# ikergarcia1996/AI-Generated-GTAV

Measured on AMD Instinct MI355X. Metric: generated frames/sec (32-frame clip, 100 noise steps), higher is better.
Workload: dtype fp16 (fp32 accumulate/residual)

## Files before the change

### ai-generated-gtav_amd/csrc/api_dit.hip

```cpp
#include "api_internal.h"

#ifdef GTAV_EXPERIMENTS
static int fold_alloc(gtav_dit* h) {
    gtav_dit::Fold& f = h->fold;
    if (f.ok) return 0;
    GTAV_REQUIRE(f.geom_ok, "dit_set_fold: this geometry has no LayerNorm fold (tokens per frame %d must be a multiple of 16 and >= 64, hidden %% 256 == 0)", h->P);
    Arena& a = h->arena;
    const int D = h->D;
    const size_t Mx = round_up(h->Mmax, 128);
    int rc = 0;
#define A_(expr) do { if (!rc) rc = (expr); } while (0)
    {
        const int nhb = h->L * 2, nseam = 2 * nhb + 1;
        f.col_c.assign(nseam, 0);
        int col = 0;
        for (int hb = 0; hb < nhb; ++hb) { f.col_c[2 * hb + 1] = col; col += 2 * h->Hm; }
        for (int hb = 0; hb < nhb; ++hb) { f.col_c[2 * hb] = col; col += 2 * 3 * D; }
        f.col_c[2 * nhb] = col; col += 2 * h->Nfin;
        f.CTW = col;
        f.n_groups = 2 * nseam; f.n_groups_a = 2 * nhb;
        f.Rp = round_up(h->max_rows, 128);
        A_(a.alloc_t(&f.ctab, (size_t)h->max_rows * f.CTW));
        A_(a.alloc_t(&f.ctab_cur, (size_t)h->maxB * h->maxT * f.CTW));
        A_(a.alloc_t(&f.stats, Mx * (size_t)(D / 64) * 2));
// ... 46 lines not shown
static int dit_fold_tables(gtav_dit* h, int rows, bool fa, bool fb, hipStream_t s) {
    if (!fa && !fb) return 0;
#ifndef GTAV_EXPERIMENTS
    (void)h; (void)rows; (void)s;
    GTAV_REQUIRE(false, "the LayerNorm fold exists only in the experiments build");
#else
    gtav_dit::Fold& f = h->fold;
    const int ng = fb ? f.n_groups : f.n_groups_a;
    RET_IF(launch_ctab_inputs(h->mod, h->MODW, rows, round_up(rows, 128), h->D, f.gcol_dev, f.gscale_dev, ng, f.sx, (size_t)f.Rp * h->D, s));
    return launch_gemm_grouped(f.groups_dev, ng, h->Hm > 3 * h->D ? h->Hm : 3 * h->D, rows, h->D, s);
#endif
}
static void fold_consumer(const gtav_dit* h, GemmParams& q, int seam, int N, const int* mod_rows, const float* ctab) {
    const gtav_dit::Fold& fo = h->fold;
    q.bias = nullptr;
    q.f_P = h->P; q.f_rows = mod_rows; q.f_stats = fo.stats; q.f_nslot = h->D / 64;
    q.f_c1 = ctab + fo.col_c[seam]; q.f_c2 = q.f_c1 + N; q.f_ldc = fo.CTW;
}
static int fold_producer(gtav_dit* h, int cls, const f16* X, const f16* Wt, int M, int K, const float* bias, const ResidGate& gt, const float* next_scale, hipStream_t s) {
    GemmParams q = gemm_params(X, K, Wt, M, h->D, K);
    q.out = h->resid; q.ldo = h->D; q.bias = bias; q.err_flag = h->err_flag;
    q.gate = gt.gate; q.gate_stride = gt.stride; q.gate_rows = gt.rows; q.rows_per_gate = gt.rows_per_gate;
    q.f_P = h->P; q.f_rows = gt.rows; q.f_scale = next_scale; q.f_stats_out = h->fold.stats; q.f_a = h->xn;
    PROF(h, cls, s, launch_gemm(q, EPI_RESID_FOLD, s));
    return 0;
}

static int dit_cond_mlp(gtav_dit* h, int rows, bool have_actions, hipStream_t s) {
    const int ldhc = h->D + h->Apad;
    RET_IF(launch_skinny_f32(h->E, 256, h->w_t0, h->b_t0, h->HC, ldhc, rows, h->D, 256, 1, s));
    RET_IF(launch_skinny_f32(h->HC, ldhc, h->w_t2cat, have_actions ? h->b_t2a : h->b_t2, h->Sc, h->D, rows, h->D, ldhc, 1, s));
    return launch_skinny_f32(h->Sc, h->D, h->w_ada, h->b_ada, h->mod, h->MODW, rows, h->MODW, h->D, 0, s);
}

static int dit_cond(gtav_dit* h, const int64_t* t64, int rows, int Tq, const StepParams* sp, int use_cur, const float* actions,
                    int64_t act_outer, int64_t act_inner, hipStream_t s) {
    GTAV_REQUIRE(rows <= h->max_rows, "conditioning rows %d exceed max_cond_rows %d", rows, h->max_rows);
    RET_IF(launch_cond_inputs(t64, rows, Tq, sp, use_cur, h->sincos, h->E, actions, act_outer, act_inner, h->A, h->HC, h->D + h->Apad,
                              h->D, h->Apad, h->err_flag, s));
    RET_IF(dit_cond_mlp(h, rows, actions != nullptr, s));
    bool fa, fb;
    fold_policy(h, rows * h->P, fa, fb);
    return dit_fold_tables(h, rows, fa, fb, s);
}

struct DitPrefetch {
    const gtav_dit* h;
    int M, Tq, t0;
    bool on;
    DitPrefetch(const gtav_dit* h_, int M_, int Tq_, int t0_) : h(h_), M(M_), Tq(Tq_), t0(t0_) {
        const int pf_max_m = 1536;
        static const int pf_min_m = GTAV_ENV_INT("GTAV_PF_MIN_M", 256);
        on = h->w_prefetch && M >= pf_min_m && M <= pf_max_m;
    }
    PrefetchDesc after(int hb, int pos) const {
        const int q = pos + 1, hb2 = hb + q / 4, consumer = (q + 3) % 4;
        if (!on || hb2 >= 2 * h->L) return kNoPrefetch;
        const int v = h->w_prefetch_cls[consumer];
        if (!v) return kNoPrefetch;
        const gtav_dit::Half& w2 = h->halves[hb2];
        const int D = h->D;
        const f16* W; int N, K, sk = 1;
        if (consumer == 3) { W = dit_half_fused(h, hb2, M, Tq, t0) ? w2.w_qkv_hm : w2.w_qkv; N = 3 * D; K = D; }
        else if (consumer == 0) { W = w2.w_out; N = D; K = D; sk = gemm_choose_splitk(M, D, D); }
        else if (consumer == 1) { W = w2.w_fc1; N = h->Hm; K = D; }
        else { W = w2.w_fc2; N = D; K = h->Hm_pad; sk = gemm_choose_splitk(M, D, h->Hm_pad); }
        const int nkt = K / 64;
        if (sk < 1 || nkt % sk || (sk >= 8 ? sk % 8 : 8 % sk)) sk = 1;
        return PrefetchDesc{W, cdiv(N, 128), nkt, sk, v >= 2 ? v : 0};
    }
};

static bool dit_resid_inplace(const gtav_dit* h, int M, int K) {
    return gemm_pp_ok(M, h->D, K, EPI_RESID) || (gemm_choose_splitk(M, h->D, K) == 1 && M >= h->resid_inplace_min_m) || gemm_resid_inplace_ok(M, h->D, K, h->P);
}

static int dit_forward_core(gtav_dit* h, const float* x_src, const int* frame_index, int B, int Tq, int t0,
                            const float* mod, const int* mod_rows, const float* ctab, float* v_out, hipStream_t s) {
    const int D = h->D, P = h->P, NB = B * Tq, M = NB * P;
    GTAV_REQUIRE(M <= h->Mmax, "forward: %d tokens exceed workspace (%d)", M, h->Mmax);
    bool fold_a, fold_b;
    fold_policy(h, M, fold_a, fold_b);
    const DitPrefetch pf(h, M, Tq, t0);
    DeferredResid rd{h->parts, h->parts_rows * (size_t)D, h->resid, M, D, &h->prof, s};
    auto gate = [&](const float* g) { return ResidGate{g, h->MODW, mod_rows, P}; };
    auto ln = [&](const OperandOps& o, const float* shift, const float* scale, int* ef) -> int {
        PROF(h, PC_LN, s, o.ln_modulate(h->resid, D, h->xn, D, M, D, shift, scale, h->MODW, mod_rows, P, rd.take(), ef, s));
        return 0;
    };
    const int g_embed = 2 * h->L, g_final = 2 * h->L + 1;
    PROF(h, PC_OTHER, s, h->ops(g_embed).patchify(x_src, frame_index, NB, h->C, h->H, h->W, h->p, h->xp, h->Kpe, 1.f, 0.f, h->err_of(g_embed), s));
    GemmParams pe = gemm_params(h->xp, h->Kpe, h->w_pe, M, D, h->Kpe);
    pe.bias = h->b_pe; pe.out = h->resid; pe.ldo = D;
    PROF(h, PC_OTHER, s, h->ops(g_embed).gemm(pe, EPI_F32, s));
    bool folded_in = false;
    for (int hb = 0; hb < 2 * h->L; ++hb) {
        const int l = hb / 2, hf = hb % 2;
        const gtav_dit::Half& w = h->halves[hb];
        const OperandOps& ops = h->ops(hb);
        int* const ef = h->err_of(hb);
        const float* mb = mod + (size_t)hb * 6 * D;
        const bool fused = dit_half_fused(h, hb, M, Tq, t0), fused_t = fused && hf == 1, fused_s = fused && hf == 0 && !folded_in;
        if (fused_t) rd.permute_rows(Tq, P);
        if (!folded_in) RET_IF(ln(ops, mb, mb + D, ef));
        GemmParams g = gemm_params(h->xn, D, fused_t || fused_s ? w.w_qkv_hm : w.w_qkv, M, 3 * D, D);
        g.D = D; g.S = P; g.err_flag = ef; g.pf = pf.after(hb, 0);
        if (folded_in) fold_consumer(h, g, 2 * hb, 3 * D, mod_rows, ctab);
        if (hf == 0) { g.qkv_mode = QKV_SPATIAL; g.rope_cs = h->rope_s.cs_dev; }
        else { g.qkv_mode = QKV_TEMPORAL; g.k = h->kvcache[l]; g.v = h->kvcache[l]; g.Tq = Tq; g.t0 = t0; g.Tmax = h->maxT; g.rope_cs = h->rope_t.cs_dev; }
        if (fused_t || fused_s) {
            g.out = h->ao; g.ldo = D;
            if (fused_t) PROF(h, PC_ATTN_T, s, launch_gemm_qkvt_attn(g, s));
            else PROF(h, PC_ATTN_S, s, launch_gemm_qkvs_attn(g, s));
        } else {
            if (hf == 0) { g.q = h->qs; g.k = h->ks; g.v = h->vts; }
            else g.q = h->qt;
            PROF(h, PC_QKV, s, ops.gemm(g, folded_in ? EPI_QKV_FOLD : EPI_QKV, s));
            if (hf == 0) PROF(h, PC_ATTN_S, s, ops.attn_spatial(h->qs, h->ks, h->vts, h->ao, NB, h->heads, P, s, false));
            else PROF(h, PC_ATTN_T, s, ops.attn_temporal(h->qt, h->kvcache[l], h->ao, B, P, D, Tq, t0, h->maxT, s));
        }
        folded_in = false;
        GemmParams fc1 = gemm_params(h->xn, D, w.w_fc1, M, h->Hm, D);
        fc1.bias = w.b_fc1; fc1.out = h->hbuf; fc1.ldo = h->Hm_pad; fc1.err_flag = ef; fc1.pf = pf.after(hb, 2);
        if (fold_a) {
            RET_IF(fold_producer(h, PC_OUT, h->ao, w.w_out, M, D, w.b_out, gate(mb + 2 * D), mb + 4 * D, s));
            fold_consumer(h, fc1, 2 * hb + 1, h->Hm, mod_rows, ctab);
            PROF(h, PC_FC1, s, launch_gemm(fc1, EPI_GELU_TANH_FOLD, s));
        } else {
            RET_IF(rd.gemm(ops, PC_OUT, h->ao, D, w.w_out, D, w.b_out, gate(mb + 2 * D), dit_resid_inplace(h, M, D), pf.after(hb, 1)));
            RET_IF(ln(ops, mb + 3 * D, mb + 4 * D, ef));
            PROF(h, PC_FC1, s, ops.gemm(fc1, EPI_GELU_TANH, s));
        }
        if (fold_b) {
            const float* next_scale = hb + 1 < 2 * h->L ? mod + (size_t)(hb + 1) * 6 * D + D : mod + (size_t)h->L * 12 * D + D;
            RET_IF(fold_producer(h, PC_FC2, h->hbuf, w.w_fc2, M, h->Hm_pad, w.b_fc2, gate(mb + 5 * D), next_scale, s));
            folded_in = true;
        } else {
            RET_IF(rd.gemm(ops, PC_FC2, h->hbuf, h->Hm_pad, w.w_fc2, h->Hm_pad, w.b_fc2, gate(mb + 5 * D), dit_resid_inplace(h, M, h->Hm_pad), pf.after(hb, 3)));
        }
    }
    const float* mf = mod + (size_t)h->L * 12 * D;
    if (!folded_in) RET_IF(ln(h->ops(g_final), mf, mf + D, h->err_of(g_final)));
    GemmParams fin = gemm_params(h->xn, D, h->w_final, M, h->Nfin, D);
    fin.bias = h->b_final; fin.out = h->fo; fin.ldo = h->Nfin;
    if (folded_in) fold_consumer(h, fin, 4 * h->L, h->Nfin, mod_rows, ctab);
    PROF(h, PC_OTHER, s, h->ops(g_final).gemm(fin, folded_in ? EPI_F32_FOLD : EPI_F32, s));
    PROF(h, PC_OTHER, s, launch_unpatchify(h->fo, h->Nfin, v_out, NB, h->C, h->H, h->W, h->p, 0, 1.f, 0.f, s));
    return h->prof.collect(s);
}

extern "C" {

int gtav_dit_create(const gtav_dit_config* c, gtav_dit** out) {
    GTAV_REQUIRE(c && out, "dit_create: null argument");
    GTAV_REQUIRE(c->hidden_size % 256 == 0 && c->hidden_size <= 2048, "hidden_size=%d must be a multiple of 256, <= 2048", c->hidden_size);
    GTAV_REQUIRE(c->num_heads > 0 && c->hidden_size / c->num_heads == 64 && c->hidden_size % c->num_heads == 0,
                 "only head_dim 64 is implemented (hidden %d, heads %d)", c->hidden_size, c->num_heads);
    GTAV_REQUIRE(c->input_h % c->patch_size == 0 && c->input_w % c->patch_size == 0, "input %dx%d not divisible by patch %d",
                 c->input_h, c->input_w, c->patch_size);
    GTAV_REQUIRE(c->max_frames >= 1 && c->max_frames <= 32, "max_frames=%d must be in [1, 32]", c->max_frames);
    GTAV_REQUIRE(c->max_batch >= 1 && c->depth >= 1, "bad max_batch/depth");
    RET_IF(skinny_init());
    gtav_dit* h = new gtav_dit();
    h->cfg = *c;
    h->D = c->hidden_size; h->L = c->depth; h->heads = c->num_heads; h->C = c->in_channels; h->p = c->patch_size;
    h->H = c->input_h; h->W = c->input_w; h->gh = h->H / h->p; h->gw = h->W / h->p; h->P = h->gh * h->gw;
    const int D = h->D;
    if ((h->P % 8) != 0) {
        set_error("tokens per frame P=%d must be a multiple of 8", h->P);
        delete h;
        return 2;
    }
    h->Hm = (int)(D * c->mlp_ratio); h->Hm_pad = round_up(h->Hm, 128);
    h->A = c->external_cond_dim > 0 ? c->external_cond_dim : 0; h->Apad = round_up(h->A > 0 ? h->A : 1, 32);
    h->MODW = h->L * 12 * D + 2 * D;
    h->Kpe = round_up(h->C * h->p * h->p, 64);
    h->Nfin = h->p * h->p * h->C;
    h->maxB = c->max_batch; h->maxT = c->max_frames; h->Mmax = h->maxB * h->maxT * h->P;
    h->max_rows = c->max_cond_rows > h->maxB * h->maxT ? c->max_cond_rows : h->maxB * h->maxT;
    Arena& a = h->arena;
    WeightTable& wt = h->wt;
    int rc = 0;
#define A_(expr) do { if (!rc) rc = (expr); } while (0)
    A_(a.alloc_t(&h->w_pe, (size_t)round_up(D, 128) * h->Kpe));
    h->n_groups = 2 * h->L + 2;
    h->grp_bf16.assign(h->n_groups, 0);
    wt.add_f16("x_embedder.proj.weight", D, h->C * h->p * h->p, h->w_pe, round_up(D, 128), h->Kpe, 2 * h->L);
    A_(a.alloc_t(&h->b_pe, D)); wt.add_f32("x_embedder.proj.bias", 1, D, h->b_pe, D);
    A_(a.alloc_t(&h->w_t0, (size_t)D * 256)); wt.add_f32("t_embedder.mlp.0.weight", D, 256, h->w_t0, 256);
    A_(a.alloc_t(&h->b_t0, D)); wt.add_f32("t_embedder.mlp.0.bias", 1, D, h->b_t0, D);
    const int ldhc = D + h->Apad;
// ... 237 lines not shown
    GTAV_REQUIRE(t_cur >= 0 && t_cur < 1000 && t_next >= 0 && t_next < 1000 && t_ctx >= 0 && t_ctx < 1000, "denoise_step: timestep out of range");
    GTAV_REQUIRE(!actions || h->A > 0, "denoise_step: model has no external_cond");
    GTAV_REQUIRE(mode == 0 || mode == 1, "denoise_step: mode %d", mode);
    const bool prepared = cond_step >= 0;
    if (prepared)
        GTAV_REQUIRE(h->prepared.valid && h->prepared.B == B && h->prepared.F == F && h->prepared.start == start &&
                         h->prepared.cur == cur && cond_step < h->prepared.n_steps && h->prepared.actions == actions,
                     "denoise_step: cond_step=%d but gtav_dit_prepare_frame was not called for this window", cond_step);
    else
        h->prepared.valid = false;
    if (mode == 1) {
        GTAV_REQUIRE(h->kvrec.valid && h->kvrec.B == B && h->kvrec.F == F && h->kvrec.start == start && h->kvrec.cur == cur &&
                         h->kvrec.x == (const void*)x,
                     "denoise_step: context-cached step (mode 1) on window [%d, %d] without a preceding full-window step (mode 0) "
                     "on the same batch / window / latent buffer: the temporal K/V caches would be stale", start, cur);
    } else {
        h->kvrec.valid = true; h->kvrec.B = B; h->kvrec.F = F; h->kvrec.start = start; h->kvrec.cur = cur; h->kvrec.x = x;
    }
    hipStream_t s = (hipStream_t)stream;
    StepParams sp;
    sp.first = start; sp.cur = cur; sp.t_ctx = t_ctx; sp.t_cur = t_cur; sp.is_final = is_final != 0;
    sp.alpha_t = h->ac_host[t_cur]; sp.alpha_next = h->ac_host[t_next]; sp.cond_step = cond_step;
    RET_IF(launch_step_setup(h->step_dev, sp, h->frame_idx, h->mod_rows_dev, prepared ? h->mod_last : nullptr, h->mod_changed, B, mode == 1 ? 1 : T, T, F,
                             mode == 1, s));
    if (prepared) RET_IF(launch_gather_rows(h->mod, h->mod_rows_dev, h->mod_changed, h->mod_cur, B * (mode == 1 ? 1 : T), h->MODW,
                                            h->prepared.fold_tables ? h->fold.ctab : nullptr, h->fold.ctab_cur, h->fold.CTW, s));
    hipGraphExec_t exec = nullptr;
    if (h->use_graph && !h->prof.on) RET_IF(dit_step_graph(h, x, B, F, T, actions, mode, v_out, prepared, &exec));
    if (!exec) return denoise_step_body(h, x, B, F, T, actions, mode, v_out, prepared, s);
    GTAV_CHECK_HIP(hipGraphLaunch(exec, s));
    return 0;
}

int gtav_dit_set_graph(gtav_dit* h, int32_t enable) {
    GTAV_REQUIRE(h, "dit_set_graph: null handle");
    h->use_graph = enable != 0;
    return 0;
}

int gtav_dit_set_weight_prefetch(gtav_dit* h, int32_t enable) {
    GTAV_REQUIRE(h, "dit_set_weight_prefetch: null handle");
    GTAV_REQUIRE(enable == 0 || enable == 1 || (enable >> 16) == 1,
                 "dit_set_weight_prefetch: mode %d (0 off, 1 on, 0x10000 | per-class nibbles: bits 0-3 out-proj's weight, 4-7 fc1's, 8-11 fc2's, 12-15 to_qkv's; "
                 "nibble 0 = not prefetched, 1 = the whole slice, k >= 2 = the first k K tiles of every row tile)", enable);
    int cls[4];
    for (int c = 0; c < 4; ++c) cls[c] = enable == 0 ? 0 : enable == 1 ? 1 : (enable >> (4 * c)) & 15;
    const bool on = cls[0] || cls[1] || cls[2] || cls[3];
    if (h->w_prefetch != on || memcmp(cls, h->w_prefetch_cls, sizeof(cls))) h->drop_graphs();
    h->w_prefetch = on;
    memcpy(h->w_prefetch_cls, cls, sizeof(cls));
    return 0;
}

#ifdef GTAV_EXPERIMENTS
int gtav_dit_set_fold(gtav_dit* h, int32_t mode, int32_t min_tokens_a, int32_t min_tokens_b) {
    GTAV_REQUIRE(h && mode >= 0 && mode <= 2, "dit_set_fold: mode %d", mode);
    if (min_tokens_a >= 0) h->fold.min_m_a = min_tokens_a;
    if (min_tokens_b >= 0) h->fold.min_m_b = min_tokens_b;
    if (mode == 2 || (mode == 1 && (h->fold.min_m_a < (1 << 30) || h->fold.min_m_b < (1 << 30)))) RET_IF(fold_alloc(h));
    h->drop_graphs();
    h->prepared.valid = false;
    h->fold.mode = mode;
    return 0;
}
#endif

static int dit_set_fused(gtav_dit* h, bool& flag, int hf, bool geom_ok, bool enable) {
    if (flag != enable) h->drop_graphs();
    if (enable && geom_ok) {
        for (int l = 0; l < h->L; ++l) {
            gtav_dit::Half& w = h->halves[l * 2 + hf];
            if (w.w_qkv_hm) continue;
            RET_IF(h->arena.alloc_t(&w.w_qkv_hm, (size_t)3 * h->D * h->D));
            if (h->finalized) RET_IF(launch_qkv_head_major(w.w_qkv, w.w_qkv_hm, h->D, nullptr, hf ? 0 : 1));
        }
        if (h->finalized) GTAV_CHECK_HIP(hipDeviceSynchronize());
    }
    flag = enable;
    return 0;
}
int gtav_dit_set_fused_temporal(gtav_dit* h, int32_t enable) {
    GTAV_REQUIRE(h, "dit_set_fused_temporal: null handle");
    return dit_set_fused(h, h->fuse_tattn, 1, h->P % 16 == 0 && h->D % 256 == 0 && h->maxT >= 5, enable != 0);
}
int gtav_dit_set_fused_spatial(gtav_dit* h, int32_t enable) {
    GTAV_REQUIRE(h, "dit_set_fused_spatial: null handle");
    return dit_set_fused(h, h->fuse_sattn, 0, h->P == 144 && h->D % 256 == 0, enable != 0);
}

int gtav_dit_fused_launches(gtav_dit* h, int32_t B, int32_t T, int32_t t0) {
    if (!h || B < 1 || T < 1) return 0;
    int mask = 0;
    for (int hb = 0; hb < 2 * h->L; ++hb)
        if (dit_half_fused(h, hb, B * T * h->P, T, t0)) mask |= (hb & 1) ? 2 : 1;
    return mask;
}

int gtav_dit_profile(gtav_dit* h, int32_t enable) {
    GTAV_REQUIRE(h, "dit_profile: null handle");
    h->prof.reset(enable != 0);
    return 0;
}
int gtav_dit_profile_read(gtav_dit* h, double* ms_by_class, int64_t* launches_by_class) {
    GTAV_REQUIRE(h && ms_by_class && launches_by_class, "dit_profile_read: null argument");
    h->prof.read(ms_by_class, launches_by_class);
    return 0;
// ... 74 lines not shown
```

### ai-generated-gtav_amd/csrc/api_internal.h

```cpp
#pragma once
#include "../../include/gtav_amd.h"
#include "../../include/gtav_amd_testing.h"
#include "ops.h"
#include "ops_bf16.h"

#include <cmath>
#include <cstdarg>
#include <cstdio>
#include <cstdlib>
#include <cstring>
#include <map>
#include <string>
#include <tuple>
#include <vector>

using namespace gtav;

#define RET_IF(expr)            \
    do {                        \
        int _rc = (expr);       \
        if (_rc) return _rc;    \
    } while (0)

namespace gtav {
// ... 181 lines not shown
            GTAV_CHECK_HIP(hipEventElapsedTime(&t, ev[i], ev[i + 1]));
            ms[cls[i / 2]] += t;
            n[cls[i / 2]] += 1;
        }
        used = 0;
        return 0;
    }
    void reset(bool enable) {
        on = enable;
        used = 0;
        for (int i = 0; i < PC_COUNT; ++i) { ms[i] = 0; n[i] = 0; }
    }
    void read(double* ms_by_class, int64_t* launches_by_class) const {
        for (int i = 0; i < PC_COUNT; ++i) { ms_by_class[i] = ms[i]; launches_by_class[i] = n[i]; }
    }
    ~Profiler() {
        for (hipEvent_t e : ev) (void)hipEventDestroy(e);
    }
};
#define PROF(h, c, s, expr)            \
    do {                               \
        RET_IF((h)->prof.begin(c, s)); \
        RET_IF(expr);                  \
        RET_IF((h)->prof.end(s));      \
    } while (0)

inline int report_err_flag(int flag, const char* who) {
    GTAV_REQUIRE(!(flag & ERR_TIMESTEP), "%s: a timestep outside [0, 999] was passed", who);
    GTAV_REQUIRE(!(flag & ERR_NONFINITE), "%s: a NaN or inf was found in the input tensor", who);
    GTAV_REQUIRE(!(flag & ERR_F16_SAT), "%s: an activation exceeded the fp16 range (|x| > 65504) and was saturated; results since the "
                 "last check are finite but clipped (the reference runs this path in bf16, which has fp32 range)", who);
    return 0;
}

inline GemmParams gemm_params(const f16* X, int ldx, const f16* W, int M, int N, int K) {
    GemmParams g;
    memset(&g, 0, sizeof(g));
    g.X = X; g.ldx = ldx; g.W = W; g.M = M; g.N = N; g.K = K;
    return g;
}

const PrefetchDesc kNoPrefetch{nullptr, 0, 0, 0, 0};

struct ResidGate { const float* gate; int stride; const int* rows; int rows_per_gate; };
struct DeferredResid {
    float* parts; size_t parts_floats;
    float* resid;
    int M, N;
    Profiler* prof;
    hipStream_t s;
    LnPending pend;
    bool pending = false;
    int gemm(const OperandOps& ops, int cls, const f16* X, int ldx, const f16* W, int K, const float* bias, const ResidGate& gt, bool inplace,
             const PrefetchDesc& pf = kNoPrefetch, float* x_out = nullptr, f16* y_save = nullptr) {
        GemmParams q = gemm_params(X, ldx, W, M, N, K);
        q.out = parts; q.ldo = N; q.pf = pf;
        if (inplace) {
            q.out = resid; q.bias = bias; q.gate = gt.gate; q.gate_stride = gt.stride; q.gate_rows = gt.rows; q.rows_per_gate = gt.rows_per_gate;
        } else {
            q.splitk = gemm_choose_splitk(M, N, K);
            GTAV_REQUIRE((size_t)q.splitk * M * N <= parts_floats, "split-K slabs exceed workspace");
        }
        if (prof) RET_IF(prof->begin(cls, s));
        RET_IF(ops.gemm(q, inplace ? EPI_RESID : EPI_PARTIAL, s));
        if (prof) RET_IF(prof->end(s));
        pending = !inplace;
        if (inplace) return 0;
        memset(&pend, 0, sizeof(pend));
        pend.parts = parts; pend.nsplit = q.splitk; pend.slab_stride = (size_t)M * N; pend.ld = N; pend.bias = bias;
        pend.gate = gt.gate; pend.gate_stride = gt.stride; pend.gate_rows = gt.rows; pend.rows_per_gate = gt.rows_per_gate;
        pend.x_out = x_out; pend.y_save = y_save;
        return 0;
    }
    const LnPending* take() {
        const bool was = pending;
        pending = false;
        return was ? &pend : nullptr;
    }
    void permute_rows(int T, int P) {
        if (!pending) memset(&pend, 0, sizeof(pend));
        pend.tperm_T = T; pend.tperm_P = P;
        pending = true;
    }
    void save_shift(float* k) { pend.k_save = k; }
    int load_shift(const float* k) {
        GTAV_REQUIRE(!pending, "train_block_forward: a re-run starts from a stored block input");
        memset(&pend, 0, sizeof(pend));
        pend.k_load = k;
        pending = true;
        return 0;
    }
};

}
}
using namespace gtav::api;

struct gtav_dit {
    Profiler prof;
    gtav_dit_config cfg;
    int D, L, heads, P, gh, gw, C, p, H, W, Hm, Hm_pad, A, Apad, MODW, Kpe, Nfin, maxB, maxT, Mmax, max_rows;
    Arena arena;
    WeightTable wt;
    f16 *w_pe = nullptr, *w_final = nullptr;
    struct Half { f16 *w_qkv, *w_out, *w_fc1, *w_fc2; float *b_out, *b_fc1, *b_fc2; f16* w_qkv_hm; };
    std::vector<Half> halves;
    float *b_pe = nullptr, *b_final = nullptr;
    float *w_t0, *b_t0, *w_t2cat, *b_t2, *b_ext, *b_t2a, *w_ada, *b_ada;
    float* sincos = nullptr;
    bool sincos_set = false;
    RopeTable rope_s, rope_t;
    std::vector<float> freqs_s, freqs_t;
    float *freqs_s_dev = nullptr, *freqs_t_dev = nullptr;
    f16 *xp, *xn, *qs, *ks, *vts, *qt, *ao, *hbuf;
    std::vector<f16*> kvcache;
    float *resid, *fo, *vout, *E, *HC, *Sc, *mod, *parts;
    size_t parts_rows = 0;
    int* err_flag = nullptr;
    std::vector<unsigned char> grp_bf16;
    int n_groups = 0;
    bool any_bf16 = false;
    const OperandOps& ops(int g) const { return operand_ops(grp_bf16[g] != 0); }
    int* err_of(int g) const { return err_flag + 4 + g; }
    int* frame_idx = nullptr;
    StepParams* step_dev = nullptr;
    int* mod_rows_dev = nullptr;
    float* mod_cur = nullptr;
    int *mod_last = nullptr, *mod_changed = nullptr;
    int* t_steps_dev = nullptr;
    struct { bool valid = false, fold_tables = false; int B = 0, F = 0, start = 0, cur = 0, n_steps = 0; const float* actions = nullptr; } prepared;
    struct { bool valid = false; int B = 0, F = 0, start = 0, cur = 0; const void* x = nullptr; } kvrec;
    struct GraphKey {
        int B, F, T, mode;
        const void *x, *actions, *vout;
        bool operator<(const GraphKey& o) const {
            return std::tie(B, F, T, mode, x, actions, vout) < std::tie(o.B, o.F, o.T, o.mode, o.x, o.actions, o.vout);
        }
    };
    std::map<GraphKey, hipGraphExec_t> graphs;
    bool use_graph = true;
    bool fuse_tattn = false;
    bool fuse_sattn = false;
    bool w_prefetch = true;
    int w_prefetch_cls[4] = {1, 4, 4, 1};
    int resid_inplace_min_m = GTAV_ENV_INT("GTAV_RESID_INPLACE_MIN_M", 1 << 30);
    struct Fold {
        bool geom_ok = false;
        bool ok = false;
        int mode = 1;
        int min_m_a = 1 << 30, min_m_b = 1 << 30;
        int CTW = 0, n_groups = 0, n_groups_a = 0, Rp = 0;
        std::vector<int> col_c;
        float *ctab = nullptr, *ctab_cur = nullptr, *stats = nullptr;
        f16* sx = nullptr;
        GemmGroup* groups_dev = nullptr;
        int *gcol_dev = nullptr, *gscale_dev = nullptr;
    } fold;
    hipStream_t cap_stream = nullptr;
    void drop_graphs() {
        for (auto& kv : graphs)
            if (kv.second) (void)hipGraphExecDestroy(kv.second);
        graphs.clear();
    }
    ~gtav_dit() {
        drop_graphs();
        if (cap_stream) (void)hipStreamDestroy(cap_stream);
    }
    float* ac_table = nullptr;
    std::vector<float> ac_host;
    bool finalized = false;
    struct Train {
        bool on = false, have_fwd = false, have_actions = false;
        bool bf16 = false;
        int window = 8;
        bool recompute = false;
        int rc_block = -1;
        std::vector<float*> kshift;
        size_t saved_bytes = 0;
        int B = 0, T = 0, M = 0, Mp = 0, rows = 0;
        float loss_scale = 65536.0f;
        float grad_div = 1.0f;
        std::vector<Slot*> params;
        struct Linear { Slot *w = nullptr, *b = nullptr; };
        struct HalfSlots { Linear qkv, out, fc1, fc2, ada; };
        std::vector<HalfSlots> hs;
        Linear fin, fin_ada, pe, t0, t2, ext;
        float* grad_arena = nullptr;
        size_t grad_count = 0;
        float* ctl = nullptr;
        float *ln_part = nullptr;
        float *red_ws = nullptr, *sumsq_part = nullptr;
        size_t red_ws_floats = 0;
        AdamParam* adam_params = nullptr;
        AdamItem* adam_items = nullptr;
        int adam_n_items = 0;
        std::vector<float*> res;
        struct HB { f16 *xnA, *ao, *y1, *xnB, *u, *hh, *y2, *q, *k, *v; };
// ... 10 lines not shown
```

### ai-generated-gtav_amd/csrc/elementwise.hip

```cpp
#include "ops.h"

#include <cstdlib>
#include <type_traits>

#include <cstring>

namespace gtav {

namespace {

template <int MODE, int NV>
__global__ __launch_bounds__(256) void ln_wave_row_kernel(const float* __restrict__ x, int ldx, f16* __restrict__ out, int M, int D,
                                                          const float* __restrict__ p0, const float* __restrict__ p1, int mod_stride,
                                                          const int* __restrict__ rows, int rows_per_mod, int flags, int* err_flag) {
    const int lane = threadIdx.x & 63;
    const int m = blockIdx.x * 4 + (threadIdx.x >> 6);
    if (m >= M) return;
    const float* xr = x + (size_t)m * ldx;
    f32x4 v[NV], av[NV], bv[NV];
#pragma unroll
    for (int i = 0; i < NV; ++i) v[i] = *(const f32x4*)(xr + i * 256 + lane * 4);
    const float *a, *b;
    if (MODE == 0) {
        int row = m / rows_per_mod;
        if (rows) row = rows[row];
        a = p1 + (size_t)row * mod_stride;
        b = p0 + (size_t)row * mod_stride;
    } else {
        a = p0;
        b = p1;
    }
#pragma unroll
    for (int i = 0; i < NV; ++i) {
        av[i] = *(const f32x4*)(a + i * 256 + lane * 4);
        bv[i] = *(const f32x4*)(b + i * 256 + lane * 4);
    }
    const float kshift = __builtin_bit_cast(float, __builtin_amdgcn_readfirstlane(__builtin_bit_cast(int, v[0][0])));
    float s1 = 0.f, s2 = 0.f;
#pragma unroll
    for (int i = 0; i < NV; ++i) {
        const float a0 = v[i][0] - kshift, a1 = v[i][1] - kshift, a2 = v[i][2] - kshift, a3 = v[i][3] - kshift;
        s1 += (a0 + a1) + (a2 + a3);
        s2 += (a0 * a0 + a1 * a1) + (a2 * a2 + a3 * a3);
    }
    const float t1 = wave_sum_dpp(s1), t2 = wave_sum_dpp(s2);
    const float m1 = t1 / (float)D;
    const float var = fmaxf(t2 / (float)D - m1 * m1, 0.f);
    const float rstd = 1.0f / sqrtf(var + 1e-6f);
    float amax = 0.f;
#pragma unroll
    for (int i = 0; i < NV; ++i) {
        float yv[4];
#pragma unroll
        for (int e = 0; e < 4; ++e) {
            const float xh = ((v[i][e] - kshift) - m1) * rstd;
            if (MODE == 0) {
                const float sc = av[i][e] + 1e-6f;
                yv[e] = xh * (1.0f + sc) + bv[i][e];
            } else {
                yv[e] = xh * av[i][e] + bv[i][e];
            }
        }
        store_f16x4_paired<1>(out + tiled_off(m, i * 256 + lane * 4, D), sat4(yv[0], yv[1], yv[2], yv[3], amax), lane, flags & 2);
    }
    sat_report(amax, err_flag);
}

#ifdef GTAV_EXPERIMENTS
#define LN_DBG(pd, b) ((pd).flags & (b))
#else
#define LN_DBG(pd, b) false
#endif
template <int MODE, bool PEND, int KS = 0>
__global__ __launch_bounds__(512) void ln_row_block_kernel(float* __restrict__ x, int ldx, f16* __restrict__ out, int M, int D,
                                                           const float* __restrict__ p0, const float* __restrict__ p1,
                                                           int mod_stride, const int* __restrict__ rows, int rows_per_mod,
                                                           LnPending pd) {
    __shared__ float red[16];
    const int m = blockIdx.x;
    const int c = threadIdx.x * 4;
    const int nw = (blockDim.x + 63) >> 6, wid = threadIdx.x >> 6, lane = threadIdx.x & 63;
    float* xr = x + (size_t)m * ldx;
    const bool act = c < D;
    const bool nt = PEND && (pd.flags & 4);
    f32x4 v = f32x4{0.f, 0.f, 0.f, 0.f}, av = v, bv = v;
    if (act) v = nt ? __builtin_nontemporal_load((const f32x4*)(xr + c)) : *(const f32x4*)(xr + c);
    f32x4 sl[8];
    int nchunk = 0;
    if (PEND && act) {
        const float* pp = pd.parts + (size_t)m * pd.ld + c;
        auto slab = [&](int sp) -> f32x4 {
            const f32x4* q = (const f32x4*)(pp + (size_t)sp * pd.slab_stride);
            return nt ? __builtin_nontemporal_load(q) : *q;
        };
        nchunk = pd.nsplit <= 1 ? 1 : pd.nsplit <= 2 ? 2 : pd.nsplit <= 4 ? 4 : 8;
        if (nchunk == 1) {
            sl[0] = slab(0);
        } else if (nchunk == 2) {
#pragma unroll
            for (int sp = 0; sp < 2; ++sp) sl[sp] = slab(sp < pd.nsplit ? sp : 0);
        } else if (nchunk == 4) {
#pragma unroll
            for (int sp = 0; sp < 4; ++sp) sl[sp] = slab(sp < pd.nsplit ? sp : 0);
        } else {
#pragma unroll
            for (int sp = 0; sp < 8; ++sp) sl[sp] = slab(sp < pd.nsplit ? sp : 0);
        }
    }
    int row = 0, gr = 0;
    if (MODE == 0) {
        row = m / rows_per_mod;
        if (rows && !LN_DBG(pd, 0x2000)) row = rows[row];
    }
    if (PEND && pd.gate) {
        gr = m / pd.rows_per_gate;
        if (pd.gate_rows && !LN_DBG(pd, 0x2000)) gr = pd.gate_rows[gr];
    }
    const float kshift = LN_DBG(pd, 0x200) ? 0.f : KS == 2 ? pd.k_load[m] : xr[0];
    if (act && !LN_DBG(pd, 0x100)) {
        av = *(const f32x4*)((MODE == 0 ? p1 + (size_t)row * mod_stride : p0) + c);
        bv = *(const f32x4*)((MODE == 0 ? p0 + (size_t)row * mod_stride : p1) + c);
    }
    if (PEND && act) {
        f32x4 y = pd.bias && !LN_DBG(pd, 0x100) ? *(const f32x4*)(pd.bias + c) : f32x4{0.f, 0.f, 0.f, 0.f};
        f32x4 g4 = f32x4{1.f, 1.f, 1.f, 1.f};
        if (pd.gate && !LN_DBG(pd, 0x100)) g4 = *(const f32x4*)(pd.gate + (size_t)gr * pd.gate_stride + c);
#pragma unroll
        for (int sp = 0; sp < 8; ++sp)
            if (sp < nchunk && sp < pd.nsplit) y = y + sl[sp];
        if (pd.y_save) {
            float am = 0.f;
// ... 520 lines not shown
                else v = ((const float*)src)[(((size_t)f * 3 + c) * H + (y0 + a)) * W + (x0 + j)];
                row += aa_w(x0 + j, cx, ix) * v;
            }
            acc += wy * row;
        }
        dst[idx] = acc / (wxs * wys) * in_scale;
    }
}

inline int grid_for(size_t total, int block = 256) {
    size_t g = (total + block - 1) / block;
    if (g > 256 * 16) g = 256 * 16;
    if (g < 1) g = 1;
    return (int)g;
}

__global__ void qkv_head_major_kernel(const f16* __restrict__ src, f16* __restrict__ dst, int D, int mode) {
    const size_t i = (size_t)blockIdx.x * blockDim.x + threadIdx.x;
    const int cpr = D >> 3;
    if (i >= (size_t)3 * D * cpr) return;
    const int nd = (int)(i / cpr), kc = (int)(i - (size_t)nd * cpr);
    const int hd = nd / 192, rem = nd - hd * 192;
    int which, d;
    if (mode == 0) {
        which = rem >> 6;
        d = rem & 63;
    } else {
        const int w = rem / 48, r48 = rem - w * 48;
        which = r48 >> 4;
        d = 16 * w + (r48 & 15);
    }
    const int ns = which * D + hd * 64 + d;
    *(uint4*)(dst + tiled_off(nd, kc * 8, D)) = *(const uint4*)(src + tiled_off(ns, kc * 8, D));
}

__global__ void calib_spin_kernel(unsigned long long ticks, unsigned long long* __restrict__ dev_ticks) {
    const unsigned long long t0 = __builtin_amdgcn_s_memrealtime();
    unsigned long long t1 = t0;
    while (t1 - t0 < ticks) {
        __builtin_amdgcn_s_sleep(2);
        t1 = __builtin_amdgcn_s_memrealtime();
    }
    if (threadIdx.x == 0) dev_ticks[0] = t1 - t0;
}

}

static int g_ln_flags = GTAV_ENV_INT("GTAV_LN_FLAGS", 7);

static int g_ln_wave_row_min = GTAV_ENV_INT("GTAV_LN_WAVE_ROW_MIN", 0);

#define LN_WAVE_ROW_(MODE, NV, P0, P1, STRIDE, ROWS, RPM) \
    GTAV_LAUNCH((ln_wave_row_kernel<MODE, NV>), dim3(cdiv(M, 4)), dim3(256), 0, stream, x, ldx, out, M, D, P0, P1, STRIDE, ROWS, RPM, pd_.flags, err_flag)
#define LN_DISPATCH(MODE, P0, P1, STRIDE, ROWS, RPM)                                                     \
    do {                                                                                                  \
        LnPending pd_;                                                                                    \
        memset(&pd_, 0, sizeof(pd_));                                                                     \
        if (pend) pd_ = *pend;                                                                            \
        pd_.flags = g_ln_flags;                                                                           \
        pd_.err_flag = err_flag;                                                                          \
        GTAV_REQUIRE(pd_.tperm_T == 0 || (pd_.tperm_P % 16 == 0 && M % (pd_.tperm_T * pd_.tperm_P) == 0), "ln: bad output row permutation"); \
        const bool upd_ = pend && pend->parts;    \
        GTAV_REQUIRE(!pd_.k_save || (upd_ && !pd_.k_load), "ln: k_save needs a pending update and excludes k_load");                          \
        GTAV_REQUIRE(!pd_.k_load || !upd_, "ln: k_load excludes a pending update");                                                            \
        if (pd_.k_save || pd_.k_load) {                  \
            const dim3 g_(M), b_(round_up(D / 4, 64));                                                    \
            if (pd_.k_save) GTAV_LAUNCH((ln_row_block_kernel<MODE, true, 1>), g_, b_, 0, stream, x, ldx, out, M, D, P0, P1, STRIDE, ROWS, RPM, pd_); \
            else GTAV_LAUNCH((ln_row_block_kernel<MODE, false, 2>), g_, b_, 0, stream, x, ldx, out, M, D, P0, P1, STRIDE, ROWS, RPM, pd_);      \
        } else if (!upd_ && pd_.tperm_T == 0 && M >= g_ln_wave_row_min && (D == 256 || D == 512 || D == 1024 || D == 2048)) { \
            if (D == 256) LN_WAVE_ROW_(MODE, 1, P0, P1, STRIDE, ROWS, RPM);                               \
            else if (D == 512) LN_WAVE_ROW_(MODE, 2, P0, P1, STRIDE, ROWS, RPM);                          \
            else if (D == 1024) LN_WAVE_ROW_(MODE, 4, P0, P1, STRIDE, ROWS, RPM);                         \
            else LN_WAVE_ROW_(MODE, 8, P0, P1, STRIDE, ROWS, RPM);                                        \
        } else {                                                                   \
            const dim3 g_(M), b_(round_up(D / 4, 64));                                                    \
            if (upd_) GTAV_LAUNCH((ln_row_block_kernel<MODE, true>), g_, b_, 0, stream, x, ldx, out, M, D, P0, P1, STRIDE, ROWS, RPM, pd_); \
            else GTAV_LAUNCH((ln_row_block_kernel<MODE, false>), g_, b_, 0, stream, x, ldx, out, M, D, P0, P1, STRIDE, ROWS, RPM, pd_);     \
        }                                                                                                 \
    } while (0)

int launch_ln_modulate(float* x, int ldx, f16* out, int ldo, int M, int D, const float* shift, const float* scale,
                       int mod_stride, const int* rows, int rows_per_mod, const LnPending* pend, int* err_flag, hipStream_t stream) {
    GTAV_REQUIRE(D % 64 == 0 && D <= 2048 && rows_per_mod > 0 && ldo == D, "ln_modulate: D=%d must be %%64, <= 2048, ldo == D", D);
    GTAV_REQUIRE(!pend || !pend->parts || (pend->nsplit >= 1 && pend->nsplit <= 8 && pend->ld % 4 == 0 && (!pend->gate || pend->rows_per_gate > 0)),
                 "ln_modulate: bad pending update");
    LN_DISPATCH(0, shift, scale, mod_stride, rows, rows_per_mod);
    GTAV_CHECK_HIP(hipGetLastError());
    return 0;
}

int launch_ln_affine(float* x, int ldx, f16* out, int ldo, int M, int D, const float* gamma, const float* beta,
                     const LnPending* pend, int* err_flag, hipStream_t stream) {
    GTAV_REQUIRE(D % 64 == 0 && D <= 2048 && ldo == D, "ln_affine: D=%d must be %%64, <= 2048, ldo == D", D);
    GTAV_REQUIRE(!pend || !pend->parts || (pend->nsplit >= 1 && pend->nsplit <= 8 && pend->ld % 4 == 0 && (!pend->gate || pend->rows_per_gate > 0)),
                 "ln_affine: bad pending update");
    LN_DISPATCH(1, gamma, beta, 0, (const int*)nullptr, 1);
    GTAV_CHECK_HIP(hipGetLastError());
    return 0;
}
#undef LN_DISPATCH
#undef LN_WAVE_ROW_

int launch_patchify(const float* img, const int* frame_index, int NB, int C, int H, int W, int p, f16* out, int ldo,
                    float a, float b, int* err_flag, hipStream_t stream) {
    GTAV_REQUIRE(H % p == 0 && W % p == 0 && ldo >= C * p * p, "patchify: bad geometry");
    const size_t total = (size_t)NB * (H / p) * (W / p) * ldo;
    if (p % 4 == 0 && W % 4 == 0 && ldo % 4 == 0 && ((uintptr_t)img & 15) == 0 && (size_t)NB * (H / p) * (W / p) < (1u << 31)) {
        hipLaunchKernelGGL(patchify4_kernel, dim3(NB * (H / p) * (W / p)), dim3(256), 0, stream, img, frame_index, C, H, W, p, out, ldo, a, b, err_flag);
        GTAV_CHECK_HIP(hipGetLastError());
        return 0;
    }
    hipLaunchKernelGGL(patchify_kernel, dim3(grid_for(total)), dim3(256), 0, stream, img, frame_index, NB, C, H, W, p, out,
                       ldo, a, b, err_flag);
    GTAV_CHECK_HIP(hipGetLastError());
    return 0;
}

int launch_unpatchify(const float* y, int ldy, float* img, int NB, int C, int H, int W, int p, int order, float a,
                      float b, hipStream_t stream) {
    GTAV_REQUIRE(H % p == 0 && W % p == 0 && ldy >= C * p * p, "unpatchify: bad geometry");
    const size_t total = (size_t)NB * C * H * W;
    hipLaunchKernelGGL(unpatchify_kernel, dim3(grid_for(total)), dim3(256), 0, stream, y, ldy, img, NB, C, H, W, p, order,
                       a, b);
    GTAV_CHECK_HIP(hipGetLastError());
    return 0;
}

int launch_convert_pad_f16(const float* src, int lds, int R, int C, f16* dst, int Rp, int Cp, float scale, int tiled,
                           hipStream_t stream, int* err_flag) {
    GTAV_REQUIRE(Rp >= R && Cp >= C, "convert_pad: padded shape smaller than source");
// ... 206 lines not shown
```

### ai-generated-gtav_amd/csrc/gemm.hip

```cpp
#include "gemm.h"
#include "attn_tile.h"

#include <cstdlib>
#include <cstring>
#include <type_traits>
#include <hip/hip_ext.h>

namespace gtav {

namespace {

constexpr int TN = 128, TK = 64;
constexpr int TILE_BYTES = 128 * TK * 2;

typedef const __attribute__((address_space(1))) void* gptr_t;
typedef __attribute__((address_space(3))) void* lptr_t;

__device__ __forceinline__ void glds16(const char* src, char* lds_wave_base) {
    __builtin_amdgcn_global_load_lds((gptr_t)src, (lptr_t)lds_wave_base, 16, 0, 0);
}

__device__ __forceinline__ void glds16_s(const void* sbase, unsigned voff, unsigned lds_addr) {
    unsigned keep;
    asm volatile("s_mov_b32 %0, m0\n\ts_mov_b32 m0, %3\n\ts_nop 0\n\tglobal_load_lds_dwordx4 %1, %2\n\ts_mov_b32 m0, %0"
                 : "=&s"(keep) : "v"(voff), "s"(sbase), "s"(lds_addr) : "memory");
}
__device__ __forceinline__ void store16_soff(const void* sbase, unsigned voff, u32x4 v) {
    asm volatile("global_store_dwordx4 %0, %1, %2" : : "v"(voff), "v"(v), "s"(sbase) : "memory");
}
__device__ __forceinline__ void glds4_s(const void* sbase, unsigned voff, unsigned lds_addr) {
    unsigned keep;
    asm volatile("s_mov_b32 %0, m0\n\ts_mov_b32 m0, %3\n\ts_nop 0\n\tglobal_load_lds_dword %1, %2\n\ts_mov_b32 m0, %0"
                 : "=&s"(keep) : "v"(voff), "s"(sbase), "s"(lds_addr) : "memory");
}
__device__ __forceinline__ unsigned lds_offset(const void* p) { return (unsigned)(size_t)(lptr_t)p; }

__device__ __forceinline__ void store16q_sc1(void* dst, uint4 v) { store16_sc1(dst, u32x4{v.x, v.y, v.z, v.w}); }

__device__ __forceinline__ uint2 pack4(float& amax, float a, float b, float c, float d) {
    union { f16x4 h; uint2 u; } cv;
    cv.h = sat4(a, b, c, d, amax);
    return cv.u;
}


constexpr int waitcnt_imm(int vm, int lgkm) { return (vm & 15) | (7 << 4) | ((lgkm & 15) << 8) | ((vm >> 4) << 14); }
__device__ __forceinline__ f32x4 rope4(const f32x4 v, const f32x4 cs) {
    f32x4 r;
    r[0] = __builtin_fmaf(v[0], cs[0], -(v[1] * cs[1]));
    r[1] = __builtin_fmaf(v[1], cs[0], v[0] * cs[1]);
    r[2] = __builtin_fmaf(v[2], cs[2], -(v[3] * cs[3]));
    r[3] = __builtin_fmaf(v[3], cs[2], v[2] * cs[3]);
    return r;
}

__device__ __forceinline__ const float* rope_tab(const GemmParams& p, int n) { return (p.rope_cs_q && n < p.D) ? p.rope_cs_q : p.rope_cs; }

template <int VM>
__device__ __forceinline__ void wait_vm() {
    static_assert(VM >= 0 && VM < 64, "vmcnt is a 6-bit field");
    __builtin_amdgcn_s_waitcnt(waitcnt_imm(VM, 15));
}
__device__ __forceinline__ void wait_lgkm0() { __builtin_amdgcn_s_waitcnt(waitcnt_imm(63, 0)); }
__device__ __forceinline__ void wg_barrier() { asm volatile("s_barrier" ::: "memory"); }
template <int VM>
__device__ __forceinline__ void kstep_sync() {
    wait_lgkm0();
    wait_vm<VM>();
    wg_barrier();
}
template <int NS, int G>
__device__ __forceinline__ void wait_vm_ring(int rem) {
    if constexpr (NS >= 6) { if (rem >= 4) { wait_vm<4 * G>(); return; } }
    if constexpr (NS >= 5) { if (rem >= 3) { wait_vm<3 * G>(); return; } }
    if constexpr (NS >= 4) { if (rem >= 2) { wait_vm<2 * G>(); return; } }
    if constexpr (NS >= 3) { if (rem >= 1) { wait_vm<G>(); return; } }
    wait_vm<0>();
// ... 412 lines not shown
            __builtin_amdgcn_sched_barrier(0);
        }
        {
            sync(nkt - 1);
            f16x8 wf[2][FI], xf[2][FJ];
            rd(nkt - 1, wf, xf);
            per_step(nkt - 1);
            mm(wf, xf);
        }
    } else {
        for (int t = 0; t < nkt; ++t) {
            sync(t);
            const bool refill = t + NS - 1 < nkt && !GTAV_DBG(p, 1);
            if (refill && !late) stage(t + NS - 1);
            per_step(t);
            f16x8 wf[2][FI], xf[2][FJ];
            rd(t, wf, xf);
            mm(wf, xf);
            if (refill && late) {
                asm volatile("" ::: "memory");
                stage(t + NS - 1);
            }
        }
    }
}

template <bool SPLITK, int TNB, int TMB>
__device__ __forceinline__ void tile_map(const GemmParams& p, int& n0, int& m0, int& ks, int& kt0, int& nkt) {
    const int tiles_m = (p.M + TMB - 1) / TMB, tiles_n = (p.N + TNB - 1) / TNB;
    const int nwg = gridDim.x, bid = blockIdx.x;
    const int xcd = bid & 7, qq = nwg >> 3, rr = nwg & 7;
    const int swz = (xcd < rr ? xcd * (qq + 1) : rr * (qq + 1) + (xcd - rr) * qq) + (bid >> 3);
    int tile_id = swz;
    ks = 0, kt0 = 0, nkt = p.K / TK;
    if constexpr (SPLITK) {
        const int tiles = tiles_m * tiles_n;
        ks = swz / tiles;
        tile_id = swz - ks * tiles;
        nkt = nkt / p.splitk;
        kt0 = ks * nkt;
    }
    int gn = p.tm.gn;
    const int group = tiles_m * gn;
    const int ng = tile_id / group, rem = tile_id - ng * group;
    const int n_first = ng * gn;
    if (n_first + gn > tiles_n) gn = tiles_n - n_first;
    const int tile_m = rem / gn, tile_n = n_first + (rem - tile_m * gn);
    n0 = tile_n * TNB;
    m0 = tile_m * TMB;
}

__device__ __forceinline__ int div_rcp(int a, unsigned rcp) { return rcp ? (int)__umulhi((unsigned)a, rcp) : a; }
template <bool SPLITK, int TNB, int TMB>
__device__ __forceinline__ void tile_map_fast(const GemmParams& p, int& n0, int& m0, int& ks, int& kt0, int& nkt) {
    const GemmParams::TileMap& tm = p.tm;
    const int nwg = gridDim.x, bid = blockIdx.x;
    const int xcd = bid & 7, qq = nwg >> 3, rr = nwg & 7;
    const int swz = (xcd < rr ? xcd * (qq + 1) : rr * (qq + 1) + (xcd - rr) * qq) + (bid >> 3);
    int tile_id = swz;
    ks = 0, kt0 = 0, nkt = p.K / TK;
    if constexpr (SPLITK) {
        ks = div_rcp(swz, tm.rcp_tiles);
        tile_id = swz - ks * tm.tiles;
        nkt = nkt / p.splitk;
        kt0 = ks * nkt;
    }
    const int ng = div_rcp(tile_id, tm.rcp_group), rem = tile_id - ng * tm.group;
    const int n_first = ng * tm.gn;
    const bool last = n_first + tm.gn > tm.tiles_n;
    const int gn = last ? tm.tiles_n - n_first : tm.gn;
    const int tile_m = div_rcp(rem, last ? tm.rcp_gnlast : tm.rcp_gn), tile_n = n_first + (rem - tile_m * gn);
    n0 = tile_n * TNB;
    m0 = tile_m * TMB;
}

constexpr int FOLD_NFR = 4;
constexpr int fold_lds_bytes(int tnb) { return FOLD_NFR * 2 * tnb * 4; }
template <int FJ>
struct FoldTok {
    float mu[FJ], rs[FJ];
    int b1, b2, b3;
    int kmax;
    int nchunk;
    f32x4 tpre;
    const char* cb;
};
template <int FJ>
__device__ __forceinline__ int fold_frame_of(const FoldTok<FJ>& ft, int m) {
    const int k = (m >= ft.b1 ? 1 : 0) + (m >= ft.b2 ? 1 : 0) + (m >= ft.b3 ? 1 : 0);
    return k < ft.kmax ? k : ft.kmax;
}
template <int TNB, int TM, int FJ>
__device__ __forceinline__ void fold_prefetch(const GemmParams& p, int n0, int m0, int ct , int mw ,
                                              bool compute_wave, FoldTok<FJ>& ft) {
    const int mlast = m0 + TM - 1 < p.M ? m0 + TM - 1 : p.M - 1;
    const int f_first = m0 / p.f_P, nfr = mlast / p.f_P - f_first + 1;
    ft.b1 = (f_first + 1) * p.f_P; ft.b2 = ft.b1 + p.f_P; ft.b3 = ft.b2 + p.f_P;
    ft.kmax = nfr - 1;
    constexpr int Q = TNB / 4;
    ft.nchunk = nfr * 2 * Q;
    ft.tpre = f32x4{0.f, 0.f, 0.f, 0.f};
    ft.cb = nullptr;
    if (ct >= 0 && ct < ft.nchunk) {
        const int k = ct / (2 * Q), r = ct - k * 2 * Q, t = r / Q, n4 = r - t * Q;
        int n = n0 + 4 * n4;
        n = n < p.N ? n : p.N - 4;
        const int row = p.f_rows ? p.f_rows[f_first + k] : f_first + k;
        ft.tpre = *(const f32x4*)((t ? p.f_c2 : p.f_c1) + (size_t)row * p.f_ldc + n);
    }
    if (!compute_wave) return;
    const int lane = threadIdx.x & 63, li = lane & 15, g = lane >> 4;
    const int q = p.f_nslot >> 2;
    const float inv_d = 1.0f / (float)(p.f_nslot * 64);
#pragma unroll
    for (int j = 0; j < FJ; ++j) {
        int m = mw + 16 * j + li;
        m = m < p.M ? m : p.M - 1;
        const float* sp = p.f_stats + ((size_t)m * p.f_nslot + g * q) * 2;
        float a1 = 0.f, a2 = 0.f;
        if (q & 1) {
            for (int s = 0; s < q; ++s) {
                const float2 v = *(const float2*)(sp + 2 * s);
                a1 += v.x; a2 += v.y;
            }
        } else {
            for (int s = 0; s < q; s += 2) {
                const f32x4 v = *(const f32x4*)(sp + 2 * s);
// ... 936 lines not shown
    else if constexpr (FOLDC || FOLDP) epilogue<EPIX, FI, FJ, WM, 2, 0, false>(p, acc, pbias, smem, n0, m0, ks, tr, acc, ft);
    else epilogue<EPIX, FI, FJ, WM>(p, acc, pbias, smem, n0, m0, ks, tr);
    bs.end(p);
}

template <int NS, int FI, int FJ, int WM>
__global__ __launch_bounds__(128 * WM, 1) void gemm_grouped_kernel(GemmParams p0, const GemmGroup* __restrict__ groups) {
    constexpr int TNB = 32 * FI, TM = 16 * FJ * WM;
    constexpr int STAGE = (4 * FI + 2 * FJ * WM) * 1024;
    __shared__ __attribute__((aligned(16))) char smem[NS * STAGE];
    GemmParams p = p0;
    {
        const GemmGroup* gr = groups + blockIdx.y;
        p.X = gr->X; p.W = gr->W; p.out = gr->out; p.bias = gr->bias; p.N = gr->N; p.ldo = gr->ldo;
    }
    const int tiles_m = (p.M + TM - 1) / TM, tiles_n = (p.N + TNB - 1) / TNB, tiles = tiles_m * tiles_n;
    const int bid = blockIdx.x;
    if (bid >= tiles) return;
    const int xcd = bid & 7, qq = tiles >> 3, rr = tiles & 7;
    const bool inrange = (bid >> 3) < qq + (xcd < rr ? 1 : 0);
    const int tile_id = inrange ? (xcd < rr ? xcd * (qq + 1) : rr * (qq + 1) + (xcd - rr) * qq) + (bid >> 3) : bid;
    const int tile_m = tile_id / tiles_n, tile_n = tile_id - tile_m * tiles_n;
    const int n0 = tile_n * TNB, m0 = tile_m * TM;
    BlockStamps bs;
    f32x4 acc[FI][FJ];
#pragma unroll
    for (int i = 0; i < FI; ++i)
#pragma unroll
        for (int j = 0; j < FJ; ++j) acc[i][j] = f32x4{0.f, 0.f, 0.f, 0.f};
    f32x4 pbias[FI];
    auto pf = [&]() { prefetch_bias<EPI_F32, FI, WM>(p, n0, pbias); };
    mainloop_g<false, NS, FI, FJ, WM>(p, smem, n0, m0, 0, p.K / TK, acc, bs, pf);
    epilogue<EPI_F32, FI, FJ, WM>(p, acc, pbias, smem, n0, m0, 0, false);
}

template <bool TR, int NS, int FI, int FJ, int WN, int WM, int NL, int TRI = FI, bool HALFSTEP = (FI * FJ >= 16), typename AfterPrologue>
__device__ __forceinline__ void mainloop_l(const GemmParams& p, char* smem, int n0, int m0, int kt0, int nkt,
                                           f32x4 (&acc)[FI][FJ], BlockStamps& bs, AfterPrologue after_prologue) {
    static_assert(NS >= 3 && NL >= 1, "loader-wave ring: at least 3 stages and one loader wave");
    constexpr int NCW = WN * WM;
    constexpr int WPC = 2 * FI * WN, XPC = 2 * FJ * WM, NP = WPC + XPC;
    constexpr int G = (NP + NL - 1) / NL;
    constexpr int STAGE_BYTES = NP * 1024;
    const int tid = threadIdx.x, lane = tid & 63;
    const int wraw = __builtin_amdgcn_readfirstlane(tid >> 6);
    const int nktot = p.K / TK;
    if (wraw < NL) {
        const int lw = wraw;
        const int last_wt = ((p.N + 127) >> 7) - 1, last_rt = (p.M - 1) >> 7;
        const unsigned voff = (unsigned)lane * 16u;
        const unsigned smem0 = lds_offset(smem);
        const char* sb[G];
        unsigned ldso[G];
#pragma unroll
        for (int i = 0; i < G; ++i) {
            int q = lw * G + i;
            q = q < NP ? q : NP - 1;
            const bool isw = q < WPC;
            const int row = isw ? n0 + 8 * q : m0 + 8 * (q - WPC);
            int rt = row >> 7;
            const int lim = isw ? last_wt : last_rt;
            rt = rt < lim ? rt : lim;
            sb[i] = (const char*)(isw ? p.W : p.X) + ((size_t)rt * nktot + kt0) * TILE_BYTES + ((row & 127) >> 3) * 1024;
            ldso[i] = smem0 + q * 1024;
        }
        auto stage = [&](int t) {
            const unsigned so = (unsigned)(t % NS) * STAGE_BYTES;
            const size_t go = (size_t)t * TILE_BYTES;
#pragma unroll
            for (int i = 0; i < G; ++i) glds16_s(sb[i] + go, voff, ldso[i] + so);
        };
        const int npro = nkt < NS - 1 ? nkt : NS - 1;
        GTAV_STAMP_SLOT(lw == 0 && lane == 0, 7);
        for (int t = 0; t < npro; ++t) stage(t);
        for (int t = 0; t < nkt; ++t) {
            wait_vm_ring<NS, G>(nkt - 1 - t);
            GTAV_STAMP_SLOT_HI(t == 0 && lw == 0 && lane == 0, 6);
            wg_barrier();
            if (t == 0) GTAV_STAMP(bs.t[1]);
            GTAV_STAMP_SLOT(GTAV_DBG(p, 32) && lw == 0 && lane == 0 && t < 24, 8 + t);
            if (t + NS - 1 < nkt && !GTAV_DBG(p, 1)) stage(t + NS - 1);
        }
        return;
    }
    const int w = wraw - NL;
    const int wn = w % WN, wm = w / WN;
    const int li = lane & 15, g = lane >> 4;
    int woff[2], xoff[2];
#pragma unroll
    for (int s = 0; s < 2; ++s) {
        const int ch = ((4 * s + g) ^ (li & 7)) << 4;
        woff[s] = (16 * FI * wn + li) * 128 + ch;
        xoff[s] = WPC * 1024 + (16 * FJ * wm + li) * 128 + ch;
    }
    l2_prefetch_next(p, w, NCW, lane, bs.pf_sink);
    after_prologue();
    auto rd = [&](int t, f16x8 (&wf)[2][FI], f16x8 (&xf)[2][FJ]) {
        const char* b = smem + (t % NS) * STAGE_BYTES;
#pragma unroll
        for (int s = 0; s < 2; ++s) {
#pragma unroll
            for (int i = 0; i < FI; ++i) wf[s][i] = *(const f16x8*)(b + woff[s] + i * 16 * 128);
#pragma unroll
            for (int j = 0; j < FJ; ++j) xf[s][j] = *(const f16x8*)(b + xoff[s] + j * 16 * 128);
        }
    };
    auto mm = [&](const f16x8 (&wf)[2][FI], const f16x8 (&xf)[2][FJ]) {
#pragma unroll
        for (int s = 0; s < 2; ++s)
#pragma unroll
            for (int i = 0; i < FI; ++i)
#pragma unroll
                for (int j = 0; j < FJ; ++j) {
                    if (TR || i >= TRI) acc[i][j] = mfma16(xf[s][j], wf[s][i], acc[i][j], 0, 0, 0);
                    else acc[i][j] = mfma16(wf[s][i], xf[s][j], acc[i][j], 0, 0, 0);
                }
    };
    if constexpr (HALFSTEP) {
        f16x8 wa[FI], xa[FJ], wb[FI], xb[FJ];
        auto rdh = [&](int t, int sh, f16x8 (&wf)[FI], f16x8 (&xf)[FJ]) {
            const char* b = smem + (t % NS) * STAGE_BYTES;
#pragma unroll
            for (int i = 0; i < FI; ++i) wf[i] = *(const f16x8*)(b + woff[sh] + i * 16 * 128);
#pragma unroll
            for (int j = 0; j < FJ; ++j) xf[j] = *(const f16x8*)(b + xoff[sh] + j * 16 * 128);
        };
// ... 6 lines not shown
                    else acc[i][j] = mfma16(wf[i], xf[j], acc[i][j], 0, 0, 0);
                }
        };
        const bool domm = !GTAV_DBG(p, 2);
        for (int t = 0; t < nkt; ++t) {
            wait_lgkm0();
            wg_barrier();
            if (t == 0) GTAV_STAMP(bs.t[1]);
            if (t > 0) {
                rdh(t, 0, wa, xa);
                if (domm) mmh(wb, xb);
                interleave_mfma_dsread<FI * FJ, FI + FJ>();
            } else {
                rdh(t, 0, wa, xa);
            }
            __builtin_amdgcn_sched_barrier(0);
            rdh(t, 1, wb, xb);
            if (domm) mmh(wa, xa);
            interleave_mfma_dsread<FI * FJ, FI + FJ>();
            __builtin_amdgcn_sched_barrier(0);
        }
        if (domm) mmh(wb, xb);
    } else {
        f16x8 wA[2][FI], xA[2][FJ], wB[2][FI], xB[2][FJ];
        auto step = [&](int t, f16x8 (&wr)[2][FI], f16x8 (&xr)[2][FJ], const f16x8 (&wm_)[2][FI], const f16x8 (&xm_)[2][FJ]) {
            GTAV_STAMP_SLOT(GTAV_DBG(p, 32) && w == 0 && lane == 0 && t < 24, 32 + t);
            wait_lgkm0();
            wg_barrier();
            if (t == 0) GTAV_STAMP(bs.t[1]);
            if (t > 0 && !GTAV_DBG(p, 2)) {
                rd(t, wr, xr);
                mm(wm_, xm_);
                interleave_mfma_dsread<2 * FI * FJ, 2 * (FI + FJ), 1>();
            } else {
                rd(t, wr, xr);
            }
            __builtin_amdgcn_sched_barrier(0);
        };
        int t = 0;
        for (; t + 1 < nkt; t += 2) {
            step(t, wA, xA, wB, xB);
            step(t + 1, wB, xB, wA, xA);
        }
        if (t < nkt) {
            step(t, wA, xA, wB, xB);
            if (!GTAV_DBG(p, 2)) mm(wA, xA);
        } else if (!GTAV_DBG(p, 2)) {
            mm(wB, xB);
        }
    }
}

template <int EPIX, int NS, int FI, int FJ, int WN, int WM, int NL>
__global__ __launch_bounds__(64 * (WN * WM + NL), 1) void gemm_l_kernel(GemmParams p) {
    constexpr int EPI = epi_base(EPIX);
    constexpr int TNB = 16 * FI * WN, TM = 16 * FJ * WM;
    constexpr int STAGE = (2 * FI * WN + 2 * FJ * WM) * 1024;
    constexpr int PNB = (TNB / 8 + 7) / 8 * 8 * 16, PTB = (TM / 8 + 7) / 8 * 8 * 16;
    constexpr int EPIB = (TM * PNB > TNB * PTB ? TM * PNB : TNB * PTB) + TM * 8 + (epi_is_fold_consumer(EPIX) ? fold_lds_bytes(TNB) : 0);
    extern __shared__ __attribute__((aligned(16))) char smem_l[];
    static_assert(NS * STAGE >= EPIB, "the ring must cover the epilogue's LDS image");
    char* smem = smem_l;
#define GTAV_PIN_S(x) asm volatile("" ::"s"(x))
    GTAV_PIN_S(p.X); GTAV_PIN_S(p.W); GTAV_PIN_S(p.M); GTAV_PIN_S(p.N); GTAV_PIN_S(p.K); GTAV_PIN_S(p.splitk);
    GTAV_PIN_S(p.tm.tiles_m); GTAV_PIN_S(p.tm.tiles_n); GTAV_PIN_S(p.tm.gn); GTAV_PIN_S(p.tm.group); GTAV_PIN_S(p.tm.tiles);
    GTAV_PIN_S(p.tm.rcp_tiles); GTAV_PIN_S(p.tm.rcp_group); GTAV_PIN_S(p.tm.rcp_gn); GTAV_PIN_S(p.tm.rcp_gnlast);
    GTAV_PIN_S(p.bias); GTAV_PIN_S(p.out); GTAV_PIN_S(p.ldo); GTAV_PIN_S(p.qkv_mode); GTAV_PIN_S(p.D);
#undef GTAV_PIN_S
    BlockStamps bs;
    bs.begin(p);
    int n0, m0, ks, kt0, nkt;
    tile_map_fast<EPI == EPI_PARTIAL, TNB, TM>(p, n0, m0, ks, kt0, nkt);
    f32x4 acc[FI][FJ];
#pragma unroll
    for (int i = 0; i < FI; ++i)
#pragma unroll
        for (int j = 0; j < FJ; ++j) acc[i][j] = f32x4{0.f, 0.f, 0.f, 0.f};
    bool tr = false;
    f32x4 pbias[FI];
    constexpr bool FOLDC = epi_is_fold_consumer(EPIX), FOLDP = EPI == EPI_RESID_FOLD;
    FoldTok<FJ> ft;
    auto pff = [&]() {
        if constexpr (FOLDC) {
            const int cw = (int)(threadIdx.x >> 6) - NL;
            fold_prefetch<TNB, TM, FJ>(p, n0, m0, (int)threadIdx.x - 64 * NL, __builtin_amdgcn_readfirstlane(m0 + 16 * FJ * (cw / WN)), cw >= 0, ft);
        }
    };
    if constexpr (EPI == EPI_QKV && FI * FJ <= 6 && WN * WM + NL <= 12) {
        tr = (p.qkv_mode == QKV_SPATIAL) && (n0 >= 2 * p.D);
        f32x4 prope[FI][FJ];
        auto pfq = [&]() {
            prefetch_bias<EPI, FI, WM, WN, NL>(p, n0, pbias);
            prefetch_rope<FI, FJ, WM, WN, NL>(p, n0, m0, prope);
            pff();
        };
        if (tr) mainloop_l<true, NS, FI, FJ, WN, WM, NL>(p, smem, n0, m0, kt0, nkt, acc, bs, pfq);
        else mainloop_l<false, NS, FI, FJ, WN, WM, NL>(p, smem, n0, m0, kt0, nkt, acc, bs, pfq);
        GTAV_STAMP(bs.t[2]);
        epilogue<EPIX, FI, FJ, WM, WN, NL, true>(p, acc, pbias, smem, n0, m0, ks, tr, prope, ft);
    } else if constexpr (EPI == EPI_QKV) {
        tr = (p.qkv_mode == QKV_SPATIAL) && (n0 >= 2 * p.D);
        auto pf = [&]() { prefetch_bias<EPI, FI, WM, WN, NL>(p, n0, pbias); pff(); };
        if (tr) mainloop_l<true, NS, FI, FJ, WN, WM, NL>(p, smem, n0, m0, kt0, nkt, acc, bs, pf);
        else mainloop_l<false, NS, FI, FJ, WN, WM, NL>(p, smem, n0, m0, kt0, nkt, acc, bs, pf);
        GTAV_STAMP(bs.t[2]);
        epilogue<EPIX, FI, FJ, WM, WN, NL, false>(p, acc, pbias, smem, n0, m0, ks, tr, acc, ft);
    } else if constexpr (FOLDP) {
        f32x4 xpre[FI][FJ];
        auto pf = [&]() { prefetch_bias<EPI, FI, WM, WN, NL>(p, n0, pbias); prefetch_resid<FI, FJ, WM, WN, NL>(p, n0, m0, xpre, 0, FI * FJ); };
        mainloop_l<false, NS, FI, FJ, WN, WM, NL>(p, smem, n0, m0, kt0, nkt, acc, bs, pf);
        GTAV_STAMP(bs.t[2]);
        epilogue<EPIX, FI, FJ, WM, WN, NL, true>(p, acc, pbias, smem, n0, m0, ks, tr, xpre, ft);
    } else {
        auto pf = [&]() { prefetch_bias<EPI, FI, WM, WN, NL>(p, n0, pbias); pff(); };
        mainloop_l<false, NS, FI, FJ, WN, WM, NL>(p, smem, n0, m0, kt0, nkt, acc, bs, pf);
        GTAV_STAMP(bs.t[2]);
        epilogue<EPIX, FI, FJ, WM, WN, NL, false>(p, acc, pbias, smem, n0, m0, ks, tr, acc, ft);
    }
    bs.template end<true>(p);
}

template <int NS>
__global__ __launch_bounds__(512, 1) void gemm_qkvt_attn_kernel(GemmParams p) {
    constexpr int FI = 3, FJ = 5, WN = 4, WM = 1, NL = 4, TNB = 192, TM = 80, TMAX = 5;
    constexpr int PN = 384;
    extern __shared__ __attribute__((aligned(16))) char smem_l[];
    static_assert(NS * (2 * FI * WN + 2 * FJ * WM) * 1024 >= TM * PN, "the ring must cover the epilogue's LDS image");
    char* smem = smem_l;
#define GTAV_PIN_S(x) asm volatile("" ::"s"(x))
    GTAV_PIN_S(p.X); GTAV_PIN_S(p.W); GTAV_PIN_S(p.M); GTAV_PIN_S(p.N); GTAV_PIN_S(p.K);
    GTAV_PIN_S(p.tm.tiles_m); GTAV_PIN_S(p.tm.tiles_n); GTAV_PIN_S(p.tm.gn); GTAV_PIN_S(p.tm.group); GTAV_PIN_S(p.tm.tiles);
    GTAV_PIN_S(p.tm.rcp_group); GTAV_PIN_S(p.tm.rcp_gn); GTAV_PIN_S(p.tm.rcp_gnlast);
#undef GTAV_PIN_S
    BlockStamps bs;
    bs.begin(p);
    int n0, m0, ks, kt0, nkt;
    tile_map_fast<false, TNB, TM>(p, n0, m0, ks, kt0, nkt);
    f32x4 acc[FI][FJ];
#pragma unroll
    for (int i = 0; i < FI; ++i)
#pragma unroll
        for (int j = 0; j < FJ; ++j) acc[i][j] = f32x4{0.f, 0.f, 0.f, 0.f};
    mainloop_l<false, NS, FI, FJ, WN, WM, NL>(p, smem, n0, m0, kt0, nkt, acc, bs, []() {});
    GTAV_STAMP(bs.t[2]);
    const int tid = threadIdx.x, lane = tid & 63, w = (tid >> 6) - NL, li = lane & 15, g = lane >> 4;
    const int head = n0 / TNB;
    const int pgs = p.S >> 4, tile_m = m0 / TM, b = tile_m / pgs, pg = tile_m - b * pgs;
    float amax = 0.f;
    __syncthreads();
    if (w >= 0) {
#pragma unroll
        for (int i = 0; i < FI; ++i) {
            const int nl = 16 * FI * w + 16 * i + 4 * g;
            const bool rope = nl < 128;
            const int d = nl & 63;
#pragma unroll
            for (int j = 0; j < FJ; ++j) {
                const int ml = 16 * j + li;
                f32x4 v = acc[i][j];
                if (rope) {
                    const f32x4 cs = *(const f32x4*)(p.rope_cs + (p.t0 + j) * 64 + d);
                    v = rope4(v, cs);
                }
                char* dst = smem + ml * PN + (((nl >> 3) ^ (ml & 7)) << 4) + ((nl >> 2) & 1) * 8;
                *(uint2*)dst = pack4(amax, v[0], v[1], v[2], v[3]);
            }
        }
    }
    sat_report(amax, p.err_flag);
    __syncthreads();
    for (int q = tid; q < TM * 16 && !GTAV_DBG(p, 512); q += 512) {
        const int r = q >> 4, cc = q & 15, t = r >> 4, pl = r & 15;
        const uint4 val = *(const uint4*)(smem + r * PN + (((8 + cc) ^ (r & 7)) << 4));
        const size_t slot = ((size_t)b * p.Tmax + p.t0 + t) * p.S + 16 * pg + pl;
        f16* dst = p.k + slot * 2 * p.D + (cc >= 8 ? p.D : 0) + head * 64 + (cc & 7) * 8;
        if (p.out_sc1) store16q_sc1(dst, val);
        else *(uint4*)dst = val;
    }
    union H8 { f16x8 v; f16x2 h[4]; };
    if (tid < 3 * 128) {
        const int c = tid & 7, pl = (tid >> 3) & 15, grp = tid >> 7;
        H8 k8[TMAX], v8[TMAX];
        const int thi = TMAX - 1 - grp;
#pragma unroll
        for (int t = 0; t < TMAX; ++t) {
            if (t <= thi) {
                const int r = 16 * t + pl;
                k8[t].v = *(const f16x8*)(smem + r * PN + (((8 + c) ^ (r & 7)) << 4));
                v8[t].v = *(const f16x8*)(smem + r * PN + (((16 + c) ^ (r & 7)) << 4));
            }
        }
#pragma unroll
        for (int half = 0; half < 2; ++half) {
            const int tl = half == 0 ? thi : grp;
            if (half == 1 && grp == thi) break;
            H8 q8;
            {
                const int r = 16 * tl + pl;
                q8.v = *(const f16x8*)(smem + r * PN + ((c ^ (r & 7)) << 4));
            }
            float sc[TMAX];
            float mx = -INFINITY;
#pragma unroll
            for (int t = 0; t < TMAX; ++t) {
                sc[t] = -INFINITY;
                if (t <= tl) {
                    float dsum = 0.f;
#pragma unroll
                    for (int e = 0; e < 4; ++e) dsum = dot2acc(q8.h[e], k8[t].h[e], dsum, false);
                    sc[t] = group8_sum(dsum) * 0.125f;
                    mx = fmaxf(mx, sc[t]);
                }
            }
            float den = 0.f, o[8] = {0.f, 0.f, 0.f, 0.f, 0.f, 0.f, 0.f, 0.f};
#pragma unroll
            for (int t = 0; t < TMAX; ++t) {
                if (t <= tl) {
                    const float pr = __builtin_amdgcn_exp2f((sc[t] - mx) * 1.4426950408889634f);
                    den += pr;
#pragma unroll
                    for (int e = 0; e < 8; ++e) o[e] = __builtin_fmaf(pr, (float)v8[t].v[e], o[e]);
                }
            }
            const float inv = 1.0f / den;
            union { f16x8 h; u32x4 u; } o8;
#pragma unroll
            for (int e = 0; e < 8; ++e) o8.h[e] = (f16)(o[e] * inv);
            const int row = (b * p.Tq + tl) * p.S + 16 * pg + pl;
            store16_sc1((f16*)p.out + tiled_off(row, head * 64 + c * 8, p.D), o8.u);
        }
    }
    bs.template end<true>(p);
}


template <int NS>
__global__ __launch_bounds__(768, 1) void gemm_qkvs_attn_kernel(GemmParams p) {
    constexpr int FI = 3, FJ = 5, WN = 4, WM = 2, NL = 4, TNB = 192, TM = 144, NQT = TM / 16, NK = 10;
    constexpr int S_pad = 16 * NK, vstride = (S_pad + 8) * 2;
    constexpr int QS = 0, KS = TM * 128, VS = KS + S_pad * 128, IMG = VS + 64 * vstride;
    extern __shared__ __attribute__((aligned(16))) char smem_l[];
    static_assert(NS * (2 * FI * WN + 2 * FJ * WM) * 1024 >= IMG, "the ring must cover the epilogue's LDS image");
    static_assert(16 * FJ * WM >= TM && 16 * FJ * WM == S_pad, "two token halves cover the frame");
    char* smem = smem_l;
#define GTAV_PIN_S(x) asm volatile("" ::"s"(x))
    GTAV_PIN_S(p.X); GTAV_PIN_S(p.W); GTAV_PIN_S(p.M); GTAV_PIN_S(p.N); GTAV_PIN_S(p.K);
    GTAV_PIN_S(p.tm.tiles_m); GTAV_PIN_S(p.tm.tiles_n); GTAV_PIN_S(p.tm.gn); GTAV_PIN_S(p.tm.group); GTAV_PIN_S(p.tm.tiles);
    GTAV_PIN_S(p.tm.rcp_group); GTAV_PIN_S(p.tm.rcp_gn); GTAV_PIN_S(p.tm.rcp_gnlast);
#undef GTAV_PIN_S
    BlockStamps bs;
    bs.begin(p);
    int n0, m0, ks, kt0, nkt;
    tile_map_fast<false, TNB, TM>(p, n0, m0, ks, kt0, nkt);
    const int tid = threadIdx.x, lane = tid & 63, wraw = tid >> 6, w = wraw - NL, li = lane & 15, g = lane >> 4;
    const int wn = w & (WN - 1), wm = w >> 2;
    f32x4 acc[FI][FJ];
#pragma unroll
    for (int i = 0; i < FI; ++i)
#pragma unroll
        for (int j = 0; j < FJ; ++j) acc[i][j] = f32x4{0.f, 0.f, 0.f, 0.f};
    f32x4 cs[FJ];
    auto pf = [&]() {
#pragma unroll
        for (int j = 0; j < FJ; ++j) {
            const int pos = 16 * (FJ * wm + j) + li;
            cs[j] = *(const f32x4*)(p.rope_cs + (pos < TM ? pos : TM - 1) * 64 + 16 * wn + 4 * g);
        }
    };
    mainloop_l<false, NS, FI, FJ, WN, WM, NL, 2, true>(p, smem, n0, m0, kt0, nkt, acc, bs, pf);
    GTAV_STAMP(bs.t[2]);
    const int head = n0 / TNB, frame = m0 / TM;
    float amax = 0.f;
    __syncthreads();
    if (w >= 0) {
        const int d = 16 * wn + 4 * g;
#pragma unroll
        for (int j = 0; j < FJ; ++j) {
            const int jj = FJ * wm + j;
            if (jj < NQT) {
                const int ml = 16 * jj + li;
                const int off = ml * 128 + (((d >> 3) ^ (ml & 7)) << 4) + ((d >> 2) & 1) * 8;
                const f32x4 qv = rope4(acc[0][j], cs[j]), kv = rope4(acc[1][j], cs[j]);
                *(uint2*)(smem + QS + off) = pack4(amax, qv[0], qv[1], qv[2], qv[3]);
                *(uint2*)(smem + KS + off) = pack4(amax, kv[0], kv[1], kv[2], kv[3]);
                const f32x4 vv = acc[2][j];
                *(uint2*)(smem + VS + (16 * wn + li) * vstride + (16 * jj + 4 * g) * 2) = pack4(amax, vv[0], vv[1], vv[2], vv[3]);
            }
        }
    } else {
        for (int q = tid; q < (S_pad - TM) * 8; q += 64 * NL) *(uint4*)(smem + KS + TM * 128 + q * 16) = make_uint4(0, 0, 0, 0);
        for (int q = tid; q < 64 * (S_pad - TM) / 8; q += 64 * NL) {
            const int dd = q / ((S_pad - TM) / 8), c = q - dd * ((S_pad - TM) / 8);
            *(uint4*)(smem + VS + dd * vstride + TM * 2 + c * 16) = make_uint4(0, 0, 0, 0);
        }
    }
    sat_report(amax, p.err_flag);
    __syncthreads();
    if (GTAV_DBG(p, 64)) GTAV_STAMP(bs.t[2]);
    if (wraw < NQT) {
        const int qr = wraw * 16 + li;
        const char* qrow = smem + QS + qr * 128;
        f16x8 qf[2];
        qf[0] = *(const f16x8*)(qrow + ((g ^ (qr & 7)) << 4));
        qf[1] = *(const f16x8*)(qrow + (((4 + g) ^ (qr & 7)) << 4));
        attn_1p_tile<NK>(smem + KS, smem + VS, qf, TM, wraw * 16, (f16*)p.out, frame * TM + wraw * 16, head * 64, p.D, lane, 0);
    }
// ... 172 lines not shown
                int mm = m0 + 16 * FJ * wm + 16 * j + li_e;
                mm = mm < p.M ? mm : p.M - 1;
                gslot[j] = mm / p.rows_per_gate - gfirst;
            }
#pragma unroll
            for (int i = 0; i < FI; ++i) pbias[i] = *(const f32x4*)(garea + LP_MAXF * TNB + 16 * FI * wn + 16 * i + 4 * g4_e);
        }
#pragma unroll
        for (int i = 0; i < FI; ++i) {
            const int n = n0 + 16 * FI * wn + 16 * i + 4 * g4_e;
#pragma unroll
            for (int j = 0; j < FJ; ++j) {
                const int m = m0 + 16 * FJ * wm + 16 * j + li_e;
                const bool ok = n < p.N && m < p.M;
                const f32x4 v = acc[i][j] + pbias[i];
                if constexpr (RES) {
                    if (ok) {
                        const f32x4 gq = *(const f32x4*)(garea + gslot[j] * TNB + 16 * FI * wn + 16 * i + 4 * g4_e);
                        const f32x4 r = xres[i][j] + gq * v;
                        float* dst = (float*)p.out + (size_t)m * p.ldo + n;
                        if (p.out_sc1) store16_sc1(dst, r);
                        else *(f32x4*)dst = r;
                    }
                } else if constexpr (EPI == EPI_PARTIAL) {
                    if (ok) {
                        float* dst = (float*)p.out + (size_t)m * p.ldo + n;
                        if (p.out_sc1) store16_sc1(dst, v);
                        else *(f32x4*)dst = v;
                    }
                } else {
                    const float xin[4] = {v[0], v[1], v[2], v[3]};
                    float yo[4];
                    if constexpr (EPI == EPI_GELU_TANH) gelu_tanh_f4(xin, yo);
                    else { yo[0] = xin[0]; yo[1] = xin[1]; yo[2] = xin[2]; yo[3] = xin[3]; }
                    const uint2 mine = pack4(amax, yo[0], yo[1], yo[2], yo[3]);
                    const unsigned o0 = __shfl_xor(mine.x, 16, 64), o1 = __shfl_xor(mine.y, 16, 64);
                    if (ok && !(lane_e & 16)) {
                        f16* dst = (f16*)p.out + tiled_off(m, n, p.ldo);
                        if (p.out_sc1) store16_sc1(dst, u32x4{mine.x, mine.y, o0, o1});
                        else *(uint4*)dst = uint4{mine.x, mine.y, o0, o1};
                    }
                }
            }
        }
    }
    if constexpr (EPI != EPI_PARTIAL) sat_report(amax, p.err_flag);
}

}

static thread_local int g_force_stages = 0, g_force_wm = GTAV_ENV_INT("GTAV_GEMM_SHAPE", 0);
static int g_debug = GTAV_ENV_INT("GTAV_GEMM_DEBUG", 0);
void gemm_set_stages(int ns) { g_force_stages = ns; }
void gemm_set_wm(int wm) { g_force_wm = wm; }
#ifdef GTAV_EXPERIMENTS
void gemm_set_debug(int bits) { g_debug = bits; }
static unsigned long long* g_stamps = nullptr;
static int g_stamp_blocks = 0;
void gemm_set_stamps(unsigned long long* buf, int max_blocks) { g_stamps = buf; g_stamp_blocks = max_blocks; }
#endif

static int g_lp_enable = GTAV_ENV_INT("GTAV_LP", 1);
static int g_resid_inplace = GTAV_ENV_INT("GTAV_RESID_INPLACE", 1);
static bool lp_takes(int M, int N, int K) { return g_lp_enable && N <= 2048 && N % 8 == 0 && K >= 512 && cdiv(M, 192) * cdiv(N, 128) >= 160; }
bool gemm_resid_inplace_ok(int M, int N, int K, int rows_per_gate) {
    return g_resid_inplace && lp_takes(M, N, K) && (rows_per_gate == 0 || rows_per_gate >= 32) && (g_force_wm == 0 || g_force_wm == 31);
}
int gemm_choose_splitk(int M, int N, int K) {
    if (lp_takes(M, N, K)) return 1;
#ifdef GTAV_EXPERIMENTS
    if (g_debug & 256) return 1;
#endif
    const int tiles = cdiv(M, 128) * cdiv(N, TN);
    int s = 1;
    static const int old_rule = GTAV_ENV_INT("GTAV_SPLITK_OLD", 0);
    const int min_slice = (tiles >= 48 && !old_rule) ? 512 : 256;
    while (tiles * s < 192 && s < 8 && (K / TK) % (s * 2) == 0 && K / (s * 2) >= min_slice) s *= 2;
    if (s == 1 && K >= 4096 && (K / TK) % 2 == 0) {
        const int t192 = cdiv(M, 192) * cdiv(N, TN);
        if (t192 >= 160 && t192 < 320) s = 2;
    }
    return s;
}

#define GEMM_LAUNCH(kern, grid, block) GTAV_LAUNCH(kern, grid, block, 0, stream, p)

static int g_num_cus[64] = {0};
static int device_cus(int* dev_out) {
    int dev = 0;
    if (hipGetDevice(&dev) != hipSuccess) return 0;
    *dev_out = dev;
    if (!g_num_cus[dev & 63]) {
        int n = 0;
        if (hipDeviceGetAttribute(&n, hipDeviceAttributeMultiprocessorCount, dev) != hipSuccess || n <= 0) n = 256;
        g_num_cus[dev & 63] = n;
    }
    return g_num_cus[dev & 63];
}
static int g_l_for_8 = GTAV_ENV_INT("GTAV_L_FOR_8", 1);
#ifndef GTAV_EXPERIMENTS
bool gemm_pp_ok(int, int, int, int) { return false; }
#endif

static int g_force_gn = GTAV_ENV_INT("GTAV_GEMM_GN", 0);
static int choose_gn(int M, int N, int K, int tmb, int tnb, int splitk) {
    const int tiles_n = cdiv(N, tnb);
#ifdef GTAV_EXPERIMENTS
    if (g_debug & 1024) return tiles_n >= 8 ? tiles_n >> 3 : 1;
#endif
    if (g_force_gn < 0) return tiles_n >= 8 ? tiles_n >> 3 : 1;
    if (g_force_gn > 0) return g_force_gn < tiles_n ? g_force_gn : tiles_n;
    const double ks = (double)K / (splitk > 0 ? splitk : 1);
    const double xs = 2.0 * M * ks, ws = 2.0 * N * ks, wpanel = 2.0 * tnb * ks;
    const double c = splitk >= 8 ? 1.0 : 8.0 / (splitk > 0 ? splitk : 1);
    auto cost_of = [&](int gn) {
        const int g = cdiv(tiles_n, gn);
        return g * xs + ws * (c > g ? c / g : 1.0);
    };
    int best = 1;
    double best_cost = 1e300;
    const bool one_round = (long long)cdiv(M, tmb) * tiles_n * (splitk > 0 ? splitk : 1) <= 512;
    for (int gn = 1; gn <= tiles_n; ++gn) {
        if (!one_round && gn > 1 && gn * wpanel > 2.0 * 1024 * 1024) break;
        const double cost = cost_of(gn);
        if (cost < best_cost * 0.999) best_cost = cost, best = gn;
    }
    const int gn1 = tiles_n >= 8 ? tiles_n >> 3 : 1;
    if (best_cost > 0.8 * cost_of(gn1)) best = gn1;
    return best;
}

static int fill_tile_map(GemmParams::TileMap& tm, int M, int N, int K, int tmb, int tnb, int splitk) {
    tm.tiles_m = cdiv(M, tmb);
    tm.tiles_n = cdiv(N, tnb);
    tm.tiles = tm.tiles_m * tm.tiles_n;
    tm.gn = choose_gn(M, N, K, tmb, tnb, splitk);
    tm.group = tm.tiles_m * tm.gn;
    const int gnlast = tm.tiles_n % tm.gn ? tm.tiles_n % tm.gn : tm.gn;
    auto rcp = [](int d) { return (unsigned)((0x100000000ull + (unsigned)d - 1) / (unsigned)d); };
    GTAV_REQUIRE((long long)tm.tiles * splitk < 65536, "gemm: grid of %d tiles x %d slices is too large for the 32-bit reciprocal tile map", tm.tiles, splitk);
    tm.rcp_tiles = tm.tiles > 1 ? rcp(tm.tiles) : 0;
    tm.rcp_group = tm.group > 1 ? rcp(tm.group) : 0;
    tm.rcp_gn = tm.gn > 1 ? rcp(tm.gn) : 0;
    tm.rcp_gnlast = gnlast > 1 ? rcp(gnlast) : 0;
    return 0;
}

template <int EPI, int NS, int FI, int FJ, int WN, int WM, int NL>
static int launch_l(const GemmParams& p, int splitk, hipStream_t stream) {
    constexpr int LDS = NS * (2 * FI * WN + 2 * FJ * WM) * 1024;
    static unsigned long long attr_devs = 0;
    int dev = 0;
    GTAV_REQUIRE(device_cus(&dev) > 0, "gemm: no current device");
    if (!(attr_devs >> (dev & 63) & 1)) {
        GTAV_CHECK_HIP(hipFuncSetAttribute((const void*)gemm_l_kernel<EPI, NS, FI, FJ, WN, WM, NL>, hipFuncAttributeMaxDynamicSharedMemorySize, LDS));
        attr_devs |= 1ull << (dev & 63);
    }
    GemmParams q = p;
    if (int rc_ = fill_tile_map(q.tm, p.M, p.N, p.K, 16 * FJ * WM, 16 * FI * WN, splitk)) return rc_;
    const dim3 grid(q.tm.tiles * splitk);
    GTAV_LAUNCH((gemm_l_kernel<EPI, NS, FI, FJ, WN, WM, NL>), grid, dim3(64 * (WN * WM + NL)), LDS, stream, q);
    GTAV_CHECK_HIP(hipGetLastError());
    return 0;
}

template <int EPI, int NS, int FI = 4, int FJ = 3, int WN = 2, int WM = 4>
static int launch_lp(const GemmParams& p, hipStream_t stream) {
    constexpr int TNB = 16 * FI * WN, TM = 16 * FJ * WM;
    constexpr int LDS = NS * (TNB + TM) * 128 + (EPI == EPI_RESID ? 2 * (LP_MAXF + 1) * TNB * 4 : 0);
    if constexpr (EPI == EPI_RESID) GTAV_REQUIRE(!p.gate || (p.rows_per_gate > 0 && (TM - 1) / p.rows_per_gate + 2 <= LP_MAXF), "gemm/resid on the persistent kernel: %d tokens per gate row are too few (a tile may touch at most %d rows)", p.rows_per_gate, LP_MAXF);
    static unsigned long long attr_devs = 0;
    int dev = 0;
    const int cus = device_cus(&dev);
    GTAV_REQUIRE(cus > 0, "gemm: no current device");
    if (!(attr_devs >> (dev & 63) & 1)) {
        GTAV_CHECK_HIP(hipFuncSetAttribute((const void*)gemm_lp_kernel<EPI, NS, FI, FJ, WN, WM>, hipFuncAttributeMaxDynamicSharedMemorySize, LDS));
        attr_devs |= 1ull << (dev & 63);
    }
    GemmParams q = p;
    if (EPI == EPI_RESID && !q.gate) q.rows_per_gate = 1 << 30;
    const int T = cdiv(p.M, TM) * cdiv(p.N, TNB);
    q.tm.gn = choose_gn(p.M, p.N, p.K, TM, TNB, 1);
    GTAV_LAUNCH((gemm_lp_kernel<EPI, NS, FI, FJ, WN, WM>), dim3(T < cus ? T : cus), dim3(768), LDS, stream, q);
    GTAV_CHECK_HIP(hipGetLastError());
    return 0;
}

#ifdef GTAV_EXPERIMENTS
#include "gemm_experiments.inc"
#endif

template <int EPI>
static int launch_epi(const GemmParams& p_in, int ns, int shape, int splitk, hipStream_t stream) {
    GemmParams p = p_in;
    auto set_gn = [&](int tmb, int tnb) { p.tm.gn = choose_gn(p.M, p.N, p.K, tmb, tnb, splitk); };
    constexpr bool FOLDISH = EPI == EPI_RESID_FOLD || epi_is_fold_consumer(EPI);
    if constexpr (FOLDISH) GTAV_REQUIRE(shape == 2 || shape == 3 || shape == 11 || shape == 12 || shape == 13 || shape == 14 || shape == 20 || shape == 24 || shape == 26 || shape == 27 || shape == 28,
                                        "gemm: block shape %d has no LayerNorm-fold epilogue", shape);
    if (shape == 20) return launch_l<EPI, 4, 2, 3, 4, 2, 4>(p, splitk, stream);
    if (shape == 24) return launch_l<EPI, 4, 2, 1, 2, 3, 2>(p, splitk, stream);
    if (shape == 26) return launch_l<EPI, 4, 2, 2, 2, 3, 2>(p, splitk, stream);
#ifdef GTAV_EXPERIMENTS
    {
        bool handled = false;
        const int rc_ = launch_experiment_shape<EPI>(p, ns, shape, splitk, stream, handled);
        if (handled) return rc_;
    }
#else
    GTAV_REQUIRE(shape != 8 && shape != 9 && shape != 16 && shape != 17 && shape != 18 && shape != 21 && shape != 22 && shape != 23 && shape != 25 && shape != 27 && shape != 28 &&
                 shape != 30 && shape != 32 && shape != 33 && shape != 40 && shape != 41 && shape != 42, "gemm: block shape %d exists only in the experiments build (csrc/build.sh exp)", shape);
#endif
    GTAV_REQUIRE(!p.out2 || (EPI == EPI_F16_TILED && shape != 31), "gemm: a second output image (out2) exists for EPI_F16_TILED on the staged epilogue only (epilogue %d, block shape %d)", (int)EPI, shape);
    if (shape == 31) {
        if constexpr (EPI == EPI_GELU_TANH || EPI == EPI_PARTIAL || EPI == EPI_F16_TILED || EPI == EPI_RESID) {
// ... 23 lines not shown
        const dim3 grid(cdiv(p.M, 48) * cdiv(p.N, 64) * splitk);
        GEMM_LAUNCH((gemm_g_kernel<EPI, 4, 2, 1, 3>), grid, dim3(384));
    } else if (shape == 7) {
#ifndef GTAV_EXPERIMENTS
        if constexpr (EPI == EPI_QKV) {
            GTAV_REQUIRE(false, "gemm: the 256 x 256 tile has no QKV epilogue in the product build");
        } else
#endif
        if constexpr (!FOLDISH) {
            set_gn(256, 256);
            if (!g_force_gn && splitk == 1 && p.N <= 1024 && (size_t)p.M >= 8 * (size_t)p.N) p.tm.gn = cdiv(p.N, 256);
            const dim3 grid(cdiv(p.M, 256) * cdiv(p.N, 256) * splitk);
            GEMM_LAUNCH((gemm256_kernel<EPI>), grid, dim3(512));
        }
    } else if (shape == 3) {
        set_gn(128, TN);
        const dim3 grid(cdiv(p.M, 128) * cdiv(p.N, TN) * splitk);
        if (ns <= 2) GEMM_LAUNCH((gemm_kernel<EPI, 2, 4, 2>), grid, dim3(512));
        else GEMM_LAUNCH((gemm_kernel<EPI, 4, 4, 2>), grid, dim3(512));
    } else {
        GTAV_REQUIRE(shape == 2, "gemm: unknown block shape %d", shape);
        set_gn(128, TN);
        const dim3 grid(cdiv(p.M, 128) * cdiv(p.N, TN) * splitk);
        if (ns <= 2) GEMM_LAUNCH((gemm_kernel<EPI, 2, 2, 4>), grid, dim3(256));
        else GEMM_LAUNCH((gemm_kernel<EPI, 4, 2, 4>), grid, dim3(256));
    }
    GTAV_CHECK_HIP(hipGetLastError());
    return 0;
}

bool gemm_qkvt_attn_ok(int M, int D, int S, int Tq, int t0) {
    static const int max_blocks = GTAV_ENV_INT("GTAV_QKVT_MAX_BLOCKS", 256);
    return Tq == 5 && t0 == 0 && S % 16 == 0 && D % 64 == 0 && M % (Tq * S) == 0 && (M / 80) * (D / 64) <= max_blocks;
}
int launch_gemm_qkvt_attn(const GemmParams& p_in, hipStream_t stream) {
    GemmParams q = p_in;
    GTAV_REQUIRE(gemm_qkvt_attn_ok(q.M, q.D, q.S, q.Tq, q.t0), "gemm/qkvt_attn: unsupported geometry M=%d D=%d S=%d Tq=%d t0=%d", q.M, q.D, q.S, q.Tq, q.t0);
    GTAV_REQUIRE(q.N == 3 * q.D && q.K % TK == 0 && q.k && q.out && q.rope_cs && q.Tmax >= q.Tq, "gemm/qkvt_attn: missing buffers");
    GTAV_REQUIRE(((uintptr_t)q.X & 15) == 0 && ((uintptr_t)q.W & 15) == 0, "gemm: operands must be 16-byte aligned");
    constexpr int NS = 4, LDS = NS * 34 * 1024;
    static unsigned long long attr_devs = 0;
    int dev = 0;
    GTAV_REQUIRE(device_cus(&dev) > 0, "gemm: no current device");
    if (!(attr_devs >> (dev & 63) & 1)) {
        GTAV_CHECK_HIP(hipFuncSetAttribute((const void*)gemm_qkvt_attn_kernel<NS>, hipFuncAttributeMaxDynamicSharedMemorySize, LDS));
        attr_devs |= 1ull << (dev & 63);
    }
#ifdef GTAV_EXPERIMENTS
    q.debug = g_debug & (3 | 32 | 512);
    q.stamps = g_stamps;
#endif
    q.out_sc1 = 1;
    q.splitk = 1;
    if (int rc_ = fill_tile_map(q.tm, q.M, q.N, q.K, 80, 192, 1)) return rc_;
    GTAV_LAUNCH((gemm_qkvt_attn_kernel<NS>), dim3(q.tm.tiles), dim3(512), LDS, stream, q);
    GTAV_CHECK_HIP(hipGetLastError());
    return 0;
}

bool gemm_qkvs_attn_ok(int M, int D, int S) {
    static const int max_blocks = GTAV_ENV_INT("GTAV_QKVS_MAX_BLOCKS", 65535);
    return S == 144 && D % 64 == 0 && M > 0 && M % S == 0 && (long long)(M / S) * (D / 64) <= max_blocks;
}
int launch_gemm_qkvs_attn(const GemmParams& p_in, hipStream_t stream) {
    GemmParams q = p_in;
    GTAV_REQUIRE(gemm_qkvs_attn_ok(q.M, q.D, q.S), "gemm/qkvs_attn: unsupported geometry M=%d D=%d S=%d", q.M, q.D, q.S);
    GTAV_REQUIRE(q.N == 3 * q.D && q.K % TK == 0 && q.out && q.rope_cs && !q.rope_cs_q && !q.bias, "gemm/qkvs_attn: missing buffers (or a bias / a separate q table)");
    GTAV_REQUIRE(((uintptr_t)q.X & 15) == 0 && ((uintptr_t)q.W & 15) == 0, "gemm: operands must be 16-byte aligned");
    constexpr int NS = 3, LDS = NS * 44 * 1024;
    static unsigned long long attr_devs = 0;
    int dev = 0;
    GTAV_REQUIRE(device_cus(&dev) > 0, "gemm: no current device");
    if (!(attr_devs >> (dev & 63) & 1)) {
        GTAV_CHECK_HIP(hipFuncSetAttribute((const void*)gemm_qkvs_attn_kernel<NS>, hipFuncAttributeMaxDynamicSharedMemorySize, LDS));
        attr_devs |= 1ull << (dev & 63);
    }
#ifdef GTAV_EXPERIMENTS
    q.debug = g_debug & (3 | 32 | 64);
    q.stamps = g_stamps;
#endif
    q.splitk = 1;
    q.qkv_mode = QKV_SPATIAL;
    if (int rc_ = fill_tile_map(q.tm, q.M, q.N, q.K, 144, 192, 1)) return rc_;
    GTAV_LAUNCH((gemm_qkvs_attn_kernel<NS>), dim3(q.tm.tiles), dim3(768), LDS, stream, q);
    GTAV_CHECK_HIP(hipGetLastError());
    return 0;
}

bool gemm_tn_ok(int M, int N, int K) { return M > 0 && N > 0 && K > 0 && M % 128 == 0 && N % 128 == 0 && K % 64 == 0; }
static int g_tn_enable = GTAV_ENV_INT("GTAV_GEMM_TN", 0);
bool gemm_tn_pays(int M, int N, int K) { return g_tn_enable && gemm_tn_ok(M, N, K) && (M / 128) * (N / 128) >= 128; }
int launch_gemm_tn(const GemmParams& p_in, hipStream_t stream) {
    GemmParams p = p_in;
    GTAV_REQUIRE(gemm_tn_ok(p.M, p.N, p.K), "gemm_tn: M=%d, N=%d must be multiples of 128 and K=%d of 64", p.M, p.N, p.K);
    GTAV_REQUIRE(p.out && p.ldo >= p.N && p.ldo % 4 == 0, "gemm_tn: bad output ldo=%d", p.ldo);
    GTAV_REQUIRE(((uintptr_t)p.X & 15) == 0 && ((uintptr_t)p.W & 15) == 0, "gemm_tn: operands must be 16-byte aligned");
#ifdef GTAV_EXPERIMENTS
    p.debug = 0;
    p.stamps = g_stamps;
#endif
    p.splitk = 1;
    p.bias = nullptr; p.gate = nullptr;
    p.tm.gn = choose_gn(p.M, p.N, p.K, 128, 128, 1);
    const dim3 grid((p.M / 128) * (p.N / 128));
    GTAV_LAUNCH((gemm_tn_kernel<4>), grid, dim3(512), 0, stream, p);
    GTAV_CHECK_HIP(hipGetLastError());
    return 0;
}

bool gemm_dw_grouped_ok(const GemmDwGroup* g, int n, int K) {
    if (!g || n < 1 || n > GEMM_DW_MAX_GROUPS || K <= 0 || K % TK) return false;
    int tiles = 0;
    for (int i = 0; i < n; ++i) {
        if (g[i].M <= 0 || g[i].N <= 0 || g[i].M % 256 || g[i].N % 256 || g[i].ldo < g[i].N || g[i].ldo % 4) return false;
        tiles += (g[i].M >> 8) * (g[i].N >> 8);
    }
    int dev = 0;
    const int cus = device_cus(&dev);
    return cus > 0 && 2 * tiles >= cus && tiles <= 2 * cus && K >= 2048;
}

int launch_gemm_dw_grouped(const GemmDwGroup* g, int n, int K, int* err_flag, hipStream_t stream, bool tn) {
    GTAV_REQUIRE(g && n >= 1 && n <= GEMM_DW_MAX_GROUPS && K > 0 && K % TK == 0, "gemm_dw_grouped: bad arguments (n=%d K=%d)", n, K);
    GemmDwGroups gs;
    memset(&gs, 0, sizeof(gs));
    gs.n = n;
    for (int i = 0; i < n; ++i) {
        GTAV_REQUIRE(g[i].X && g[i].W && g[i].out && g[i].M > 0 && g[i].N > 0 && g[i].M % 256 == 0 && g[i].N % 256 == 0 && g[i].ldo >= g[i].N && g[i].ldo % 4 == 0,
                     "gemm_dw_grouped: group %d: M=%d, N=%d must be multiples of 256, ldo=%d >= N", i, g[i].M, g[i].N, g[i].ldo);
        GTAV_REQUIRE(((uintptr_t)g[i].X & 15) == 0 && ((uintptr_t)g[i].W & 15) == 0 && ((uintptr_t)g[i].out & 15) == 0, "gemm_dw_grouped: group %d: operands must be 16-byte aligned", i);
        gs.g[i] = g[i];
        gs.first[i + 1] = gs.first[i] + (g[i].M >> 8) * (g[i].N >> 8);
    }
    for (int i = n + 1; i <= GEMM_DW_MAX_GROUPS; ++i) gs.first[i] = gs.first[n];
    GemmParams p;
    memset(&p, 0, sizeof(p));
    p.K = K; p.splitk = 1; p.err_flag = err_flag; p.rows_per_gate = 1;
#ifdef GTAV_EXPERIMENTS
    p.stamps = g_stamps;
#endif
    if (tn) {
        GTAV_REQUIRE(K % 128 == 0, "gemm_dw_grouped: the transpose-free form contracts over whole 128-token row tiles (K=%d)", K);
        GTAV_LAUNCH(gemm256_dw_grouped_kernel<true>, dim3(gs.first[n]), dim3(512), 0, stream, p, gs);
    } else {
        GTAV_LAUNCH(gemm256_dw_grouped_kernel<false>, dim3(gs.first[n]), dim3(512), 0, stream, p, gs);
    }
    GTAV_CHECK_HIP(hipGetLastError());
    return 0;
}

int launch_gemm_grouped(const GemmGroup* groups_dev, int n_groups, int max_N, int M, int K, hipStream_t stream) {
    GTAV_REQUIRE(groups_dev && n_groups > 0 && n_groups < 65536 && M > 0 && max_N > 0 && K > 0 && K % TK == 0, "gemm_grouped: bad arguments");
    GemmParams p;
    memset(&p, 0, sizeof(p));
    p.M = M; p.N = max_N; p.K = K; p.splitk = 1;
    const dim3 grid(cdiv(M, 96) * cdiv(max_N, 128), n_groups);
    hipLaunchKernelGGL((gemm_grouped_kernel<4, 4, 2, 3>), grid, dim3(384), 0, stream, p, groups_dev);
    GTAV_CHECK_HIP(hipGetLastError());
    return 0;
}


int launch_gemm(const GemmParams& p_in, int epi_x, hipStream_t stream) {
    GemmParams p = p_in;
    const int epi = epi_base(epi_x);
    const bool fold_c = epi_is_fold_consumer(epi_x), fold_p = epi_x == EPI_RESID_FOLD;
    if (fold_c || fold_p) {
        GTAV_REQUIRE(p.f_P > 0 && p.f_P % 16 == 0 && p.M % p.f_P == 0, "gemm/fold: %d tokens per frame must be a multiple of 16 and divide M=%d", p.f_P, p.M);
        if (fold_c) {
            GTAV_REQUIRE(p.f_stats && p.f_c1 && p.f_c2 && p.f_ldc >= p.N && p.f_nslot == p.K / 64 && p.f_nslot % 4 == 0,
                         "gemm/fold: consumer needs the row statistics (K/64 = %d slots, a multiple of 4) and the c1 / c2 tables", p.K / 64);
            GTAV_REQUIRE(!p.bias, "gemm/fold: the bias of a fold consumer lives in its c2 table");
            if (epi == EPI_QKV) GTAV_REQUIRE(p.qkv_mode == QKV_TEMPORAL || p.S % 16 == 0, "gemm/fold: spatial QKV needs S %% 16 == 0");
        } else {
            GTAV_REQUIRE(p.gate && p.f_scale && p.f_stats_out && p.f_a && p.N % 64 == 0 && p.ldo >= p.N,
                         "gemm/fold: producer needs gate, next scale, statistics and operand buffers, N %% 64 == 0");
        }
    }
    p.debug = g_debug & (3 | 16 | 32 | 2048 | 8192 | 16384 | 0x1F0000);
    p.stamps = nullptr;
#ifdef GTAV_EXPERIMENTS
    p.stamps = g_stamps;
#endif
    p.out_sc1 = (g_debug & 8) ? 0 : 1;
    GTAV_REQUIRE(prefetch_desc_ok(p.pf), "gemm: bad prefetch descriptor (row tiles %d, K tiles %d, K slices %d)", p.pf.rt, p.pf.nkt, p.pf.splitk);
    if (g_debug & 0x800000) p.pf.next = nullptr;
    GTAV_REQUIRE(p.K > 0 && p.K % TK == 0, "gemm: K=%d must be a positive multiple of %d", p.K, TK);
    GTAV_REQUIRE(p.M > 0 && p.N > 0 && p.N % 4 == 0, "gemm: bad M=%d N=%d", p.M, p.N);
    GTAV_REQUIRE(((uintptr_t)p.X & 15) == 0 && ((uintptr_t)p.W & 15) == 0, "gemm: operands must be 16-byte aligned");
    int splitk = 1;
    if (epi == EPI_QKV) {
        GTAV_REQUIRE(p.N == 3 * p.D && p.D % 128 == 0, "gemm/qkv: N=%d must equal 3*D, D=%d %% 128 == 0", p.N, p.D);
        GTAV_REQUIRE(p.S > 0 && p.q && p.k && p.rope_cs, "gemm/qkv: missing buffers");
        if (p.qkv_mode == QKV_SPATIAL) {
            GTAV_REQUIRE(p.S % 4 == 0 && p.M % p.S == 0 && p.v, "gemm/qkv spatial: S=%d must divide M=%d, S %% 4 == 0", p.S, p.M);
        } else {
            GTAV_REQUIRE(p.Tq > 0 && p.M % (p.S * p.Tq) == 0 && p.t0 + p.Tq <= p.Tmax, "gemm/qkv temporal: bad frame geometry");
        }
    } else {
        GTAV_REQUIRE(p.out && p.ldo >= p.N && p.ldo % 4 == 0, "gemm: bad output ldo=%d", p.ldo);
        if (epi == EPI_RESID && p.gate) GTAV_REQUIRE(p.rows_per_gate > 0, "gemm/resid: rows_per_gate");
        if (epi == EPI_GELU_TANH || epi == EPI_GELU_ERF || epi == EPI_F16_TILED) GTAV_REQUIRE(p.ldo % 64 == 0, "gemm/gelu: tile-major output needs ldo %% 64 == 0");
        if (fold_p) GTAV_REQUIRE(p.splitk <= 1, "gemm/fold: the producer epilogue needs the complete sum (no split-K)");
        if (epi == EPI_PARTIAL) {
            splitk = p.splitk;
            GTAV_REQUIRE(splitk >= 1 && (p.K / TK) % splitk == 0, "gemm/partial: splitk=%d must divide K/64=%d", splitk, p.K / TK);
        }
    }
    const int blocks128 = cdiv(p.M, 128) * cdiv(p.N, TN) * splitk;
    const bool foldish = fold_c || fold_p;
    int wm = g_force_wm ? g_force_wm : (blocks128 <= 256 ? 3 : 2);
    if (!g_force_wm && blocks128 <= 256) {
        auto cost = [&](int tn, int tm) { return cdiv(cdiv(p.M, tm) * cdiv(p.N, tn) * splitk, 256) * (tn + tm); };
        int best = cost(128, 128);
        if (cost(128, 96) < best) best = cost(128, 96), wm = 9;
        const bool ok96 = p.N % 96 == 0 && epi != EPI_GELU_TANH && epi != EPI_GELU_ERF && epi != EPI_F16_TILED && !(epi == EPI_QKV && p.qkv_mode == QKV_SPATIAL);
        if (ok96 && cost(96, 96) < best) best = cost(96, 96), wm = 8;
        if (cost(64, 96) < best) best = cost(64, 96), wm = 14;
        if (cost(64, 48) < best) best = cost(64, 48), wm = 11;
    }
    if (!g_force_wm && !(g_debug & 64) && (wm == 9 || (wm == 8 && g_l_for_8))) wm = (g_debug & 128) ? 25 : 20;
#ifdef GTAV_EXPERIMENTS
    if (!g_force_wm && wm == 20 && (g_debug & 0x1000000) && !foldish && (p.K / TK / (splitk > 0 ? splitk : 1)) % 4 == 0) wm = 22;
    if (!g_force_wm && wm == 20 && (g_debug & 0x2000000) && !foldish && (p.K / TK / (splitk > 0 ? splitk : 1)) % 8 == 0) wm = 18;
#endif
    if (!g_force_wm && !(g_debug & 64)) {
        if (wm == 11) wm = 24;
        else if (wm == 14 && !(epi_x == EPI_PARTIAL && splitk >= 8)) wm = 26;
    }
    bool frame_tile = false;
    if (!g_force_wm && !foldish && !(g_debug & 64)) {
        const int t29 = cdiv(p.M, 144) * cdiv(p.N, 128) * splitk, t20 = cdiv(p.M, 96) * cdiv(p.N, 128) * splitk;
        if (t29 > 128 && t29 <= 256 && t20 > 256 && blocks128 <= 320) wm = 29, frame_tile = true;
    }
    if (!g_force_wm && wm == 2 && cdiv(p.M, 192) * cdiv(p.N, 128) * splitk >= 320) {
        wm = 12;
    }
// ... 51 lines not shown
```

### ai-generated-gtav_amd/csrc/gemm_typed.inc

```
struct GemmParams {
    const f16* X;
    int ldx;
    const f16* W;
    int M, N, K;
    int debug;
    unsigned long long* stamps;
    int* err_flag;
    int out_sc1;
    int splitk;
    const float* bias;
    void* out2;
    void* out;
    int ldo;
    const float* gate;
    int gate_stride;
    const int* gate_rows;
    int rows_per_gate;
    int qkv_mode;
    f16* q;
    f16* k;
    f16* v;
    int D;
    int S;
    int Tq;
    int t0;
    int Tmax;
    const float* rope_cs;
    const float* rope_cs_q;
    struct TileMap { int tiles_m, tiles_n, gn, group, tiles; unsigned rcp_tiles, rcp_group, rcp_gn, rcp_gnlast; } tm;
    int f_P;
    const int* f_rows;
    const float* f_stats;
    int f_nslot;
    const float* f_c1;
    const float* f_c2;
    int f_ldc;
    float* f_stats_out;
    const float* f_scale;
    f16* f_a;
    PrefetchDesc pf;
    float* sk_ws;
    int* sk_flags;
    int sk_dp, sk_r;
};
static_assert(sizeof(GemmParams) == 352, "GemmParams: every build and both operand types must see the same struct");

struct GemmGroup { const f16* X; const f16* W; float* out; const float* bias; int N; int ldo; };
int launch_gemm_grouped(const GemmGroup* groups_dev, int n_groups, int max_N, int M, int K, hipStream_t stream);

constexpr int GEMM_DW_MAX_GROUPS = 4;
struct GemmDwGroup { const f16* X; const f16* W; float* out; int M; int N; int ldo; };
static_assert(sizeof(GemmDwGroup) == 40, "GemmDwGroup: every build and both operand types must see the same struct");
bool gemm_dw_grouped_ok(const GemmDwGroup* g, int n, int K);
int launch_gemm_dw_grouped(const GemmDwGroup* g, int n, int K, int* err_flag, hipStream_t stream, bool tn = false);

// ... 12 lines not shown
```

### ai-generated-gtav_amd/generate.py

```python
from __future__ import annotations

from typing import Optional

import time

import torch

from . import lib as _lib
from .utils import alphas_cumprod as _alphas_cumprod

SCALING_FACTOR = 0.07843137255


@torch.inference_mode()
def vae_encode(x: torch.Tensor, vae, n_prompt_frames: int, scaling_factor: float = SCALING_FACTOR) -> torch.Tensor:
    B, t = x.shape[:2]
    H, W = x.shape[-2:]
    mom = vae.encode_moments(x.reshape(B * t, *x.shape[2:]), 2.0, -1.0)
    N, hw, mom_ch = mom.shape
    lat = torch.empty((N, vae.latent_dim, hw), device=mom.device, dtype=torch.float32)
    with torch.cuda.device(mom.device):
        _lib.check(_lib.load().gtav_moments_to_latents(mom.data_ptr(), lat.data_ptr(), N, hw, vae.latent_dim, mom_ch,
                                                       scaling_factor, _lib.current_stream()))
    return lat.reshape(B, t, vae.latent_dim, H // vae.patch_size, W // vae.patch_size)
# ... 24 lines not shown
    if (noise_chunks is None) == (rng is None):
        raise ValueError("generate_latents: give exactly one of noise_chunks and rng")
    dev = model.device
    B, n_prompt = x_prompt.shape[:2]
    x = torch.empty((B, total_frames, *x_prompt.shape[2:]), device=dev, dtype=torch.float32)
    x[:, :n_prompt] = x_prompt.to(dev, torch.float32)
    fsz = x[0, 0].numel()
    n_new = total_frames - n_prompt
    if rng is not None:
        draw = rng.next_draw()
        with torch.cuda.device(dev):
            if n_new > 0:
                _lib.check(_lib.load().gtav_rng_normal(x[:, n_prompt:].data_ptr(), total_frames * fsz, B * n_new, fsz, rng.seed, draw,
                                                       rng.sample0 & 0xFFFFFFFF, n_prompt, n_new, float(noise_abs_max), _lib.current_stream()))
    else:
        x[:, n_prompt:] = noise_chunks.to(dev, torch.float32)
        with torch.cuda.device(dev):
            _lib.check(_lib.load().gtav_clamp_frames(x.data_ptr(), B, total_frames, n_prompt, fsz, -float(noise_abs_max),
                                                     float(noise_abs_max), _lib.current_stream()))
    act = actions.to(dev, torch.float32).contiguous() if actions is not None else None
    model.set_schedule(_alphas_cumprod(clamp_min))
    noise_range = torch.linspace(0, 999, noise_steps + 1)
    t_of = [int(v) for v in noise_range]
    order = list(reversed(range(0, noise_steps + 1)))
    x_init = x.clone() if getattr(model, "range_policy", "report") == "auto" else None
    for attempt in range(1 + (model.n_operand_groups if x_init is not None else 0)):
        for i in range(n_prompt, total_frames):
            start = max(0, i + 1 - model.max_frames)
            if hoist_cond:
                model.prepare_frame_(B, total_frames, start, i, stabilization_level, [t_of[k] for k in order], act)
            for step, noise_idx in enumerate(order):
                cached = ctx_cache and noise_idx != noise_steps
                model.denoise_step_(x, start, i, stabilization_level, t_of[noise_idx], t_of[max(0, noise_idx - 1)],
                                    noise_idx <= 0, act, cached=cached, cond_step=step if hoist_cond else -1)
        try:
            model.check()
            break
        except _lib.GtavRangeSwitch:
            x.copy_(x_init)
    return x


PREFETCH_CLASSES = ("out", "fc1", "fc2", "qkv")


def prefetch_mode(cls) -> int:
    if not any(cls):
        return 0
    if all(v == 1 for v in cls):
        return 1
    return 0x10000 | cls[0] | cls[1] << 4 | cls[2] << 8 | cls[3] << 12


@torch.inference_mode()
def tune_weight_prefetch(model, B: int = 1, window: Optional[int] = None, steps: int = 24, rounds: int = 2, use_actions: bool = False,
                         latent_hw=None, per_class: bool = True, fused_temporal: bool = True, fused_spatial: bool = True) -> dict:
    dev = model.device
    T = int(window or model.max_frames)
    h, w = latent_hw or (model.input_h, model.input_w)
    F = T
    x0 = (torch.randn(B, F, model.in_channels, h, w, generator=torch.Generator().manual_seed(11)) * 0.5).to(dev)
    act = None
    if use_actions:
        act = torch.zeros(B, F, 25, device=dev)
        act[:, :, 3] = 1
    model.set_schedule(_alphas_cumprod(1e-4))
    ts = [999 - 7 * k for k in range(steps + 3)]

    def timed(cls) -> float:
        model.set_weight_prefetch(prefetch_mode(cls))
        x = x0.clone()
        model.prepare_frame_(B, F, 0, T - 1, 15, ts, act)
        for k in range(3):
            model.denoise_step_(x, 0, T - 1, 15, ts[k], ts[k + 1], False, act, cond_step=k)
        torch.cuda.synchronize(dev)
        t0 = time.perf_counter()
        for k in range(3, steps + 3):
            model.denoise_step_(x, 0, T - 1, 15, ts[k], ts[min(k + 1, steps + 2)], False, act, cond_step=k)
        torch.cuda.synchronize(dev)
        return (time.perf_counter() - t0) / steps * 1e3

    on, off, safe = (1, 1, 1, 1), (0, 0, 0, 0), (1, 4, 4, 1)
    starts = (on, off, safe) if per_class else (on, off)
    best = {cls: float("inf") for cls in starts}
    for _ in range(rounds):
        for cls in starts:
            best[cls] = min(best[cls], timed(cls))
    cur = min(starts, key=lambda cls: best[cls])
    cur_ms = best[cur]
    if per_class:
        for c in (2, 1, 0, 3):
            for v in (0, 4, 1):
                if v == cur[c]:
                    continue
                cand = cur[:c] + (v,) + cur[c + 1:]
                ms = min(timed(cand) for _ in range(rounds))
                if ms < cur_ms * 0.997:
                    cur, cur_ms = cand, ms
    model.set_weight_prefetch(prefetch_mode(cur))
    fused = None
    if fused_temporal and T == 5 and B * T * (h // model.patch_size) * (w // model.patch_size) <= 1280 and not getattr(model, "_trainable", False):
        was = bool(getattr(model, "_fused_temporal", False))
        t_off = t_on = float("inf")
        for _ in range(rounds):
            model.set_fused_temporal(False)
            t_off = min(t_off, timed(cur))
            model.set_fused_temporal(True)
            t_on = min(t_on, timed(cur))
        keep = t_on < t_off * 0.997
        model.set_fused_temporal(keep)
        timed(cur)
        fused = {"on_ms": round(t_on, 4), "off_ms": round(t_off, 4), "chosen": "on" if keep else "off", "was": was}
        cur_ms = min(cur_ms, t_on) if keep else cur_ms
    fused_s = None
    if fused_spatial and (h // model.patch_size) * (w // model.patch_size) == 144 and B * T >= 5 and model.hidden_size % 256 == 0 and not getattr(model, "_trainable", False):
        was = getattr(model, "_fused_spatial", None)
        was = True if was is None else bool(was)
        t_off = t_on = float("inf")
        for _ in range(rounds):
            model.set_fused_spatial(False)
            t_off = min(t_off, timed(cur))
            model.set_fused_spatial(True)
            t_on = min(t_on, timed(cur))
        keep = t_on < t_off * 0.997
        model.set_fused_spatial(keep)
        timed(cur)
        fused_s = {"on_ms": round(t_on, 4), "off_ms": round(t_off, 4), "chosen": "on" if keep else "off", "was": was}
        cur_ms = min(cur_ms, t_on) if keep else cur_ms
    model.check()
    chosen = "on" if cur == on else "off" if cur == off else "per-class"
    return {"on_ms": round(best[on], 4), "off_ms": round(best[off], 4), "chosen": chosen, "classes": dict(zip(PREFETCH_CLASSES, cur)),
            "mode": prefetch_mode(cur), "tuned_ms": round(cur_ms, 4), "fused_temporal_qkv_attention": fused, "fused_spatial_qkv_attention": fused_s}


def sample_inputs(gid: int, n_prompt: int, total_frames: int, frame_hw, latent_hw, latent_ch: int = 16, seed: int = 1000):
    g = torch.Generator().manual_seed(int(seed) + int(gid))
    frames = torch.rand(n_prompt, 3, *frame_hw, generator=g)
    noise = torch.randn(total_frames - n_prompt, latent_ch, *latent_hw, generator=g)
    return frames, noise


def shard_inputs(global_batch: int, rank: int, world: int, n_prompt: int, total_frames: int, frame_hw, latent_hw,
                 latent_ch: int = 16, seed: int = 1000):
    lo, hi = shard_batch(global_batch, rank, world)
    ins = [sample_inputs(g, n_prompt, total_frames, frame_hw, latent_hw, latent_ch, seed) for g in range(lo, hi)]
    return list(range(lo, hi)), torch.stack([f for f, _ in ins]), torch.stack([n for _, n in ins])


def generate_clip(dit, vae, frames: torch.Tensor, noise: Optional[torch.Tensor], total_frames: int, noise_steps: int,
                  actions: Optional[torch.Tensor] = None, ctx_cache: bool = False, to_uint8: bool = True, gather: bool = True, rng=None):
    n_prompt = frames.shape[1]
    x0 = vae_encode(frames.to(vae.device), vae, n_prompt)
    x = generate_latents(dit, x0, total_frames, noise_steps, noise, actions, ctx_cache=ctx_cache, rng=rng)
    xg = all_gather_latents(x) if gather else x
    out = vae_decode_frames(x, vae, to_uint8=to_uint8)
    vae.check()
    return xg, out


def shard_batch(B: int, rank: int, world: int):
    assert B % world == 0, f"global batch {B} must be divisible by world size {world}"
    per = B // world
    return rank * per, (rank + 1) * per


def all_gather_latents(x_local: torch.Tensor) -> torch.Tensor:
    import torch.distributed as dist
    if not (dist.is_available() and dist.is_initialized()) or dist.get_world_size() == 1:
        return x_local
    out = torch.empty((dist.get_world_size() * x_local.shape[0], *x_local.shape[1:]), device=x_local.device, dtype=x_local.dtype)
    dist.all_gather_into_tensor(out, x_local.contiguous())
    return out
```

### ai-generated-gtav_amd/lib.py

```python
from __future__ import annotations

import ctypes as C
import os
import subprocess

_HERE = os.path.dirname(os.path.abspath(__file__))
LIB_PATH = os.path.join(_HERE, "libgtav_amd.so")
HEADER_PATH = os.path.join(os.path.dirname(_HERE), "include", "gtav_amd.h")


class GtavError(RuntimeError):
    pass


class GtavRangeSwitch(GtavError):

    def __init__(self, msg, groups=()):
        super().__init__(msg)
        self.groups = list(groups)


def build(force: bool = False) -> str:
    src_dir = os.path.join(_HERE, "csrc")
    srcs = [os.path.join(src_dir, f) for f in os.listdir(src_dir)] + [HEADER_PATH]
# ... 12 lines not shown

class VaeConfig(C.Structure):
    _fields_ = [(n, C.c_int32) for n in ("latent_dim", "input_height", "input_width", "patch_size", "enc_dim", "enc_depth",
                                          "enc_heads", "dec_dim", "dec_depth", "dec_heads")] + [
        ("mlp_ratio", C.c_float), ("use_variational", C.c_int32), ("max_frames_per_call", C.c_int32)]


_p, _i, _f, _l = C.c_void_p, C.c_int32, C.c_float, C.c_int64
_u32, _u64 = C.c_uint32, C.c_uint64

SIGNATURES = {
    "gtav_last_error": [],
    "gtav_abi_version": [],
    "gtav_dit_create": [C.POINTER(DitConfig), C.POINTER(_p)],
    "gtav_dit_destroy": [_p],
    "gtav_dit_set_weight": [_p, C.c_char_p, _p, _l, _p],
    "gtav_dit_finalize": [_p, _p],
    "gtav_dit_get_weight": [_p, C.c_char_p, _p, _l, _p],
    "gtav_dit_forward": [_p, _p, _p, _p, _p, _i, _i, _p],
    "gtav_dit_set_schedule": [_p, C.POINTER(C.c_float), _i],
    "gtav_dit_denoise_step": [_p, _p, _i, _i, _i, _i, _i, _i, _i, _i, _p, _i, _i, _p, _p],
    "gtav_dit_prepare_frame": [_p, _i, _i, _i, _i, _i, C.POINTER(C.c_int32), _i, _p, _p],
    "gtav_dit_check": [_p, _p],
    "gtav_dit_operand_groups": [_p, C.POINTER(C.c_int32)],
    "gtav_dit_set_operand_dtype": [_p, _i, _i],
    "gtav_dit_get_operand_dtype": [_p, _i, C.POINTER(C.c_int32)],
    "gtav_dit_autorange": [_p, C.POINTER(C.c_int32), _p],
    "gtav_dit_train_param_count": [_p, C.POINTER(C.c_int64)],
    "gtav_dit_train_allow_window": [_p, _i],
    "gtav_dit_train_set_recompute": [_p, _i],
    "gtav_dit_train_saved_bytes": [_p, C.POINTER(C.c_int64)],
    "gtav_dit_train_enable": [_p, _p, _l],
    "gtav_dit_train_enable_typed": [_p, _p, _l, _i],
    "gtav_dit_set_loss_scale": [_p, _f],
    "gtav_dit_set_grad_divisor": [_p, _f],
    "gtav_dit_zero_grad": [_p, _p],
    "gtav_dit_train_forward": [_p, _p, _p, _p, _p, _i, _i, _p],
    "gtav_dit_train_backward": [_p, _p, _p, _p],
    "gtav_dit_train_backward_phases": [_p, _p, _p, _i, _i, _p],
    "gtav_dit_train_param_range": [_p, C.c_char_p, C.POINTER(C.c_int64), C.POINTER(C.c_int64)],
    "gtav_dit_get_grad": [_p, C.c_char_p, _p, _l, _p],
    "gtav_dit_train_get_residual": [_p, _i, _p, _l, _p],
    "gtav_dit_adamw_step": [_p, _f, _f, _f, _f, _f, _f, _p],
    "gtav_dit_train_stats": [_p, C.POINTER(C.c_float), _p],
    "gtav_dit_get_opt_state": [_p, C.c_char_p, _p, _p, _l, _p],
    "gtav_dit_set_opt_state": [_p, C.c_char_p, _p, _p, _l, _p],
    "gtav_dit_get_opt_step": [_p, C.POINTER(C.c_int64), C.POINTER(C.c_int64), _p],
    "gtav_dit_set_opt_step": [_p, _l, _l, _p],
    "gtav_dit_set_graph": [_p, _i],
    "gtav_dit_set_fused_temporal": [_p, _i],
    "gtav_dit_set_fused_spatial": [_p, _i],
    "gtav_dit_fused_launches": [_p, _i, _i, _i],
    "gtav_dit_set_weight_prefetch": [_p, _i],
    "gtav_dit_profile": [_p, _i],
    "gtav_dit_profile_read": [_p, C.POINTER(C.c_double), C.POINTER(C.c_int64)],
    "gtav_timer_calibrate": [_i, _i, C.POINTER(C.c_double), C.POINTER(C.c_double), _p],
    "gtav_comm_unique_id": [_p],
    "gtav_comm_init": [C.POINTER(_p), _i, _i, _p],
    "gtav_comm_allreduce_f32": [_p, _p, _l, _i, _p],
    "gtav_comm_allgather": [_p, _p, _p, _l, _p],
    "gtav_comm_destroy": [_p],
    "gtav_vae_create": [C.POINTER(VaeConfig), C.POINTER(_p)],
    "gtav_vae_destroy": [_p],
    "gtav_vae_set_weight": [_p, C.c_char_p, _p, _l, _p],
    "gtav_vae_finalize": [_p, _p],
    "gtav_vae_get_weight": [_p, C.c_char_p, _p, _l, _p],
    "gtav_vae_encode": [_p, _p, _f, _f, _p, _i, _p],
    "gtav_vae_decode": [_p, _p, _f, _p, _f, _f, _i, _p],
    "gtav_vae_check": [_p, _p],
    "gtav_vae_set_operand_dtype": [_p, _i],
    "gtav_vae_get_operand_dtype": [_p, C.POINTER(C.c_int32)],
    "gtav_vae_profile": [_p, _i],
    "gtav_vae_profile_read": [_p, C.POINTER(C.c_double), C.POINTER(C.c_int64)],
    "gtav_clamp_frames": [_p, _i, _i, _i, _i, _f, _f, _p],
    "gtav_ddim_update": [_p, _p, _p, _i, _i, _p, _p, _i, _p],
    "gtav_add_noise": [_p, _p, _p, _p, _i, _i, _f, _p],
    "gtav_vtarget": [_p, _p, _p, _p, _i, _i, _f, _p],
    "gtav_rng_normal": [_p, _l, _i, _i, _u64, _u32, _u32, _u32, _u32, _f, _p],
    "gtav_noise_window_rng": [_p, _p, _p, _p, _i, _i, _i, _u64, _u32, _u32, _f, _p],
    "gtav_vae_posterior_sample": [_p, _p, _i, _i, _i, _u64, _u32, _u32, _u32, _u32, _p],
    "gtav_op_rng_bits": [_p, _i, _i, _u64, _u32, _u32, _u32, _u32, _p],
    "gtav_mse": [_p, _l, _p, _l, _i, _i, _p, _p],
    "gtav_axpy_f32": [_p, _p, _f, _l, _p],
    "gtav_frames_to_u8": [_p, _p, _i, _i, _i, _p],
    "gtav_moments_to_latents": [_p, _p, _i, _i, _i, _i, _f, _p],
    "gtav_latents_to_tokens": [_p, _p, _i, _i, _i, _p],
    "gtav_strip_to_frames": [_p, _i, _i, _i, _p, _i, _i, _p],
    "gtav_resize_frames": [_p, _p, _i, _i, _i, _i, _i, _p],
    "gtav_op_gemm_f16": [_p, _i, _p, _p, _p, _i, _i, _i, _i, _i, _p, _i, _i, _p],
    "gtav_op_gemm_qkv": [_p, _i, _p, _p, _i, _i, _i, _p, _p, _p, _i, _i, _i, _i, _p, _p],
    "gtav_op_rope_interleave": [_p, _p, _p, _i, _p],
    "gtav_op_skinny_f32": [_p, _i, _p, _p, _p, _i, _i, _i, _i, _i, _p],
    "gtav_op_ln_modulate": [_p, _p, _i, _i, _p, _p, _i, _i, _p],
    "gtav_op_ln_affine": [_p, _p, _i, _i, _p, _p, _p],
    "gtav_op_attn_spatial": [_p, _p, _p, _p, _i, _i, _i, _p],
    "gtav_op_attn_temporal": [_p, _p, _p, _i, _i, _i, _i, _i, _i, _p],
    "gtav_op_attn_temporal_bf16": [_p, _p, _p, _i, _i, _i, _i, _i, _i, _p],
    "gtav_op_qkv_head_major": [_p, _p, _i, _p],
    "gtav_op_gemm_tn": [_p, _p, _i, _i, _i, _p, _i, _p],
    "gtav_op_gemm_dw_grouped": [_i, _p, _p, _p, _p, _p, _p, _i, _p],
    "gtav_op_attn_spatial_bwd": [_p, _p, _p, _p, _i, _i, _i, _p, _p, _p],
    "gtav_op_attn_spatial_bwd_bf16": [_p, _p, _p, _p, _i, _i, _i, _p, _p, _p],
    "gtav_op_attn_temporal_bwd": [_p, _p, _p, _i, _i, _i, _i, _i, _p, _p, _p],
    "gtav_op_attn_temporal_bwd_bf16": [_p, _p, _p, _i, _i, _i, _i, _i, _p, _p, _p],
    "gtav_op_gemm_qkvt_attn": [_p, _p, _i, _i, _i, _i, _i, _i, _p, _p, _p, _p],
    "gtav_op_qkv_head_major_spatial": [_p, _p, _i, _p],
# ... 81 lines not shown
```

### ai-generated-gtav_amd/model/dit.py

```python
from __future__ import annotations

import ctypes as C
import math
from collections import OrderedDict
from typing import Dict, Iterator, Optional

import torch

from .. import lib as _lib
from .. import weights as _w


def _rope_tables_axial(freqs: torch.Tensor, gh: int, gw: int):
    def ang(n):
        a = torch.linspace(-1, 1, steps=n)[:, None] * freqs[None, :]
        return a.repeat_interleave(2, dim=-1)
    ah, aw = ang(gh), ang(gw)
    a = torch.cat([ah[:, None, :].expand(gh, gw, -1), aw[None, :, :].expand(gh, gw, -1)], dim=-1).reshape(gh * gw, -1)
    cos, sin = torch.ones(gh * gw, 64), torch.zeros(gh * gw, 64)
    cos[:, : a.shape[1]] = a.cos()
    sin[:, : a.shape[1]] = a.sin()
    return cos.contiguous(), sin.contiguous()


# ... 186 lines not shown
        if sf is not None:
            self._spatial_freqs = sf.detach().float().cpu()
        if tf is not None:
            self._temporal_freqs = tf.detach().float().cpu()

    def initialize_weights(self):
        for k, shp in self._shapes().items():
            if k.endswith(".bias"):
                v = torch.zeros(shp)
            elif "adaLN_modulation" in k and k.startswith("blocks."):
                v = torch.zeros(shp)
            elif k.startswith("t_embedder.mlp") or k.startswith("final_layer.adaLN_modulation"):
                v = torch.randn(shp) * 0.01
            elif k == "final_layer.linear.weight":
                v = torch.randn(shp) * 0.001
            else:
                v = torch.randn(shp) * 0.02
            self._sd[k] = v
        self._dirty = True

    def _ensure(self, B: int, T: int, cond_rows: int = 0):
        if T > MAX_FRAMES:
            raise ValueError(f"a window of {T} frames: the temporal attention serves at most {MAX_FRAMES} (max_frames <= {MAX_FRAMES})")
        if self._trainable and self._train_max_frames is not None and T > self._train_max_frames:
            raise ValueError(f"a window of {T} frames on a trainable DiT constructed with train_max_frames={self._train_max_frames}: the handle's saved "
                             f"activations are sized for at most {self._train_max_frames} frames (train_max_frames <= {MAX_FRAMES})")
        if self._trainable and self._train_max_frames is None and T > TRAIN_MAX_FRAMES:
            raise ValueError(f"a window of {T} frames on a trainable DiT: the training step (backward temporal attention, adaLN-gradient reduction) is "
                             f"implemented for at most {TRAIN_MAX_FRAMES} frames; windows up to {MAX_FRAMES} need trainable=False")
        grow = (cond_rows > max(self._capacity_rows, self._capacity_b * self._capacity_t)) or T > self._capacity_t or B > self._capacity_b
        if grow and self._handle and self._trainable and self._grads is not None:
            raise RuntimeError(f"a trainable DiT cannot grow its workspace after training was enabled (batch {B} > {self._capacity_b}, window {T} > "
                               f"{self._capacity_t} or {cond_rows} conditioning rows > {max(self._capacity_rows, self._capacity_b * self._capacity_t)}): "
                               "size it with max_batch / max_frames / reserve() before the first step")
        if grow:
            self._capacity_rows = max(self._capacity_rows, cond_rows)
            self._capacity_t = max(self._capacity_t, T)
            self._capacity_b = max(self._capacity_b, B)
            self._free()
        if not self._handle:
            L = _lib.load()
            cfg = _lib.DitConfig(max_frames=self._capacity_t, max_batch=self._capacity_b,
                                 max_cond_rows=max(self._capacity_b * self._capacity_t, self._capacity_rows), **self._cfg_kwargs)
            with torch.cuda.device(self.device):
                _lib.check(L.gtav_dit_create(C.byref(cfg), C.byref(self._handle)))
                if getattr(self, "_fused_temporal", False):
                    _lib.check(L.gtav_dit_set_fused_temporal(self._handle, 1))
                if getattr(self, "_fused_spatial", None) is not None:
                    _lib.check(L.gtav_dit_set_fused_spatial(self._handle, int(self._fused_spatial)))
                if getattr(self, "_fold", None) is not None:
                    _lib.check(L.gtav_dit_set_fold(self._handle, *self._fold))
                if getattr(self, "_weight_prefetch", None) is not None:
                    _lib.check(L.gtav_dit_set_weight_prefetch(self._handle, int(self._weight_prefetch)))
                for g in sorted(self._bf16_groups):
                    _lib.check(L.gtav_dit_set_operand_dtype(self._handle, g, 1))
                if self._trainable:
                    n = C.c_int64(0)
                    _lib.check(L.gtav_dit_train_param_count(self._handle, C.byref(n)))
                    self._grads = torch.zeros(n.value, device=self.device, dtype=torch.float32)
                    if self._train_max_frames is not None:
                        _lib.check(L.gtav_dit_train_allow_window(self._handle, self._train_max_frames))
                    if self._train_recompute:
                        _lib.check(L.gtav_dit_train_set_recompute(self._handle, 1))
                    if self._train_bf16:
                        _lib.check(L.gtav_dit_train_enable_typed(self._handle, self._grads.data_ptr(), n.value, 1))
                    else:
                        _lib.check(L.gtav_dit_train_enable(self._handle, self._grads.data_ptr(), n.value))
                    _lib.check(L.gtav_dit_set_loss_scale(self._handle, self._loss_scale))
                    if self.grad_divisor != 1.0:
                        _lib.check(L.gtav_dit_set_grad_divisor(self._handle, self.grad_divisor))
            self._dirty = True
        if self._dirty:
            gh, gw = self.input_h // self.patch_size, self.input_w // self.patch_size
            sc, ss = _rope_tables_axial(self._spatial_freqs, gh, gw)
            tc, ts = _rope_tables_temporal(self._temporal_freqs, self._capacity_t)
            extra = {"tables.timestep_sincos": _timestep_table(), "tables.rope_spatial_cos": sc, "tables.rope_spatial_sin": ss,
                     "tables.rope_temporal_cos": tc, "tables.rope_temporal_sin": ts}
            self._upload(extra)
            if self._schedule is not None:
                self.set_schedule(self._schedule)

    def reserve(self, max_batch: int, max_frames: Optional[int] = None, noise_steps: int = 0):
        T = max_frames or self._capacity_t
        self._ensure(max_batch, T, cond_rows=max_batch * (T - 1 + noise_steps + 1) if noise_steps else 0)

    def forward(self, x: torch.Tensor, t: torch.Tensor, external_cond: Optional[torch.Tensor] = None) -> torch.Tensor:
        B, T, Cc, H, W = x.shape
        assert H == self.input_h and W == self.input_w, (
            f"Input image size ({H}*{W}) doesn't match model ({self.input_h}*{self.input_w}).")
        self._ensure(B, T)
        dev = self.device
        xd = x.to(dev, torch.float32).contiguous()
        td = t.to(dev, torch.int64).contiguous()
        ad = external_cond.to(dev, torch.float32).contiguous() if torch.is_tensor(external_cond) else None
        out = torch.empty_like(xd)
        with torch.cuda.device(dev):
            _lib.check(_lib.load().gtav_dit_forward(self._handle, xd.data_ptr(), td.data_ptr(), _lib.ptr(ad), out.data_ptr(),
                                                    B, T, _lib.current_stream()))
        return out

    __call__ = forward

    def forward_train(self, x: torch.Tensor, t: torch.Tensor, external_cond: Optional[torch.Tensor] = None) -> torch.Tensor:
        assert self._trainable, "construct the model with trainable=True"
        B, T, Cc, H, W = x.shape
        assert H == self.input_h and W == self.input_w
# ... 148 lines not shown
        with torch.cuda.device(self.device):
            _lib.check(_lib.load().gtav_dit_prepare_frame(self._handle, B, F, start, cur, int(t_ctx), arr, n, _lib.ptr(actions),
                                                          _lib.current_stream()))

    def denoise_step_(self, x: torch.Tensor, start: int, cur: int, t_ctx: int, t_cur: int, t_next: int, is_final: bool,
                      actions: Optional[torch.Tensor] = None, cached: bool = False, v_out: Optional[torch.Tensor] = None,
                      cond_step: int = -1):
        assert x.is_cuda and x.dtype == torch.float32 and x.is_contiguous()
        B, F = x.shape[:2]
        if cond_step < 0:
            self._ensure(B, cur - start + 1)
        with torch.cuda.device(self.device):
            _lib.check(_lib.load().gtav_dit_denoise_step(
                self._handle, x.data_ptr(), B, F, start, cur, int(t_ctx), int(t_cur), int(t_next), int(bool(is_final)),
                _lib.ptr(actions), 1 if cached else 0, int(cond_step), _lib.ptr(v_out), _lib.current_stream()))

    PROFILE_CLASSES = ("ln_modulate", "gemm_qkv", "attn_spatial", "attn_temporal", "gemm_out", "gemm_fc1", "gemm_fc2", "other",
                       "empty_event_pair")

    def profile(self, enable: bool):
        _lib.check(_lib.load().gtav_dit_profile(self._handle, int(bool(enable))))

    def profile_read(self):
        ms = (C.c_double * 9)()
        n = (C.c_int64 * 9)()
        _lib.check(_lib.load().gtav_dit_profile_read(self._handle, ms, n))
        return {k: (ms[i], n[i]) for i, k in enumerate(self.PROFILE_CLASSES)}

    def set_graph(self, enable: bool):
        _lib.check(_lib.load().gtav_dit_set_graph(self._handle, int(bool(enable))))

    def set_fused_temporal(self, enable: bool):
        self._fused_temporal = bool(enable)
        if self._handle:
            _lib.check(_lib.load().gtav_dit_set_fused_temporal(self._handle, int(self._fused_temporal)))

    def set_fused_spatial(self, enable: bool):
        self._fused_spatial = bool(enable)
        if self._handle:
            _lib.check(_lib.load().gtav_dit_set_fused_spatial(self._handle, int(self._fused_spatial)))

    def fused_launches(self, B: int, T: int, t0: int = 0) -> int:
        self._ensure(B, T)
        return int(_lib.load().gtav_dit_fused_launches(self._handle, int(B), int(T), int(t0)))

    def set_weight_prefetch(self, mode):
        mode = int(mode)
        if mode not in (0, 1) and (mode >> 16) != 1:
            raise ValueError(f"set_weight_prefetch: mode {mode:#x} is neither 0, 1 nor a per-class word (gtav_amd.generate.prefetch_mode)")
        self._weight_prefetch = mode
        if self._handle:
            _lib.check(_lib.load().gtav_dit_set_weight_prefetch(self._handle, mode))

    def set_fold(self, mode: int, min_tokens_a: int = -1, min_tokens_b: int = -1):
        if not getattr(_lib.load(), "_gtav_experiments", False):
            raise _lib.GtavError("set_fold: the LayerNorm fold exists only in the experiments build (gtav_amd.lib.load_experiments())")
        self._fold = (int(mode), int(min_tokens_a), int(min_tokens_b))
        if self._handle:
            _lib.check(_lib.load().gtav_dit_set_fold(self._handle, *self._fold))

    def set_operand_dtype(self, dtype, groups=None):
        if dtype not in (torch.float16, torch.bfloat16):
            raise ValueError(f"set_operand_dtype: {dtype} (torch.float16 or torch.bfloat16)")
        if self._train_bf16 and dtype == torch.float16:
            raise _lib.GtavError("set_operand_dtype: a bf16-trainable DiT (train_dtype=torch.bfloat16) keeps bf16 operands in every layer group")
        if self._trainable and not self._train_bf16 and dtype == torch.bfloat16:
            raise _lib.GtavError("set_operand_dtype: a trainable DiT keeps fp16 operands (its backward pass and loss scaling are fp16)")
        gs = set(range(self.n_operand_groups)) if groups is None else {int(g) for g in groups}
        if any(g < 0 or g >= self.n_operand_groups for g in gs):
            raise ValueError(f"set_operand_dtype: groups {sorted(gs)} outside [0, {self.n_operand_groups})")
        new = (self._bf16_groups | gs) if dtype == torch.bfloat16 else (self._bf16_groups - gs)
        if new == self._bf16_groups:
            return
        if self._handle:
            L = _lib.load()
            for g in sorted(new ^ self._bf16_groups):
                _lib.check(L.gtav_dit_set_operand_dtype(self._handle, g, 1 if g in new else 0))
            self._dirty = True
        self._bf16_groups = new

    def operand_dtypes(self):
        return [torch.bfloat16 if g in self._bf16_groups else torch.float16 for g in range(self.n_operand_groups)]

    def check(self):
        if not self._handle:
            return
        L = _lib.load()
        with torch.cuda.device(self.device):
            if self.range_policy != "auto" or self._trainable:
                _lib.check(L.gtav_dit_check(self._handle, _lib.current_stream()))
                return
            n = C.c_int32(0)
            _lib.check(L.gtav_dit_autorange(self._handle, C.byref(n), _lib.current_stream()))
            if n.value:
                d = C.c_int32(0)
                new = set()
                for g in range(self.n_operand_groups):
                    _lib.check(L.gtav_dit_get_operand_dtype(self._handle, g, C.byref(d)))
                    if d.value == 1:
                        new.add(g)
                switched = sorted(new - self._bf16_groups)
                self._bf16_groups = new
                self._dirty = True
                raise _lib.GtavRangeSwitch(f"DiT: an activation exceeded the fp16 range (|x| > 65504) in operand group(s) {switched}; those layers now run "
                                           "on bf16 operands (the reference's own autocast type): results since the last check are clipped — recompute them", switched)

# ... 7 lines not shown
```

### include/gtav_amd.h

```cpp
#ifndef GTAV_AMD_H
#define GTAV_AMD_H

#include <stdint.h>

#ifdef __cplusplus
extern "C" {
#endif

const char* gtav_last_error(void);
int gtav_abi_version(void);

typedef struct gtav_dit_config {
    int32_t input_h, input_w, patch_size, in_channels, hidden_size, depth, num_heads;
    float mlp_ratio;
    int32_t external_cond_dim, max_frames;
    int32_t max_batch;
    int32_t max_cond_rows;
} gtav_dit_config;

typedef struct gtav_dit gtav_dit;

int gtav_dit_create(const gtav_dit_config* cfg, gtav_dit** out);
void gtav_dit_destroy(gtav_dit* h);
int gtav_dit_set_weight(gtav_dit* h, const char* name, const float* src_dev, int64_t numel, void* stream);
int gtav_dit_finalize(gtav_dit* h, void* stream);
int gtav_dit_get_weight(gtav_dit* h, const char* name, float* dst_dev, int64_t numel, void* stream);

int gtav_dit_forward(gtav_dit* h, const float* x_dev, const int64_t* t_dev, const float* actions_dev, float* out_dev,
                     int32_t B, int32_t T, void* stream);

int gtav_dit_set_schedule(gtav_dit* h, const float* alphas_cumprod_host, int32_t n);

int gtav_dit_denoise_step(gtav_dit* h, float* x_dev, int32_t B, int32_t F, int32_t start, int32_t cur, int32_t t_ctx,
                          int32_t t_cur, int32_t t_next, int32_t is_final, const float* actions_dev, int32_t mode,
                          int32_t cond_step, float* v_out_dev, void* stream);
int gtav_dit_prepare_frame(gtav_dit* h, int32_t B, int32_t F, int32_t start, int32_t cur, int32_t t_ctx,
                           const int32_t* t_steps_host, int32_t n_steps, const float* actions_dev, void* stream);

int gtav_dit_set_graph(gtav_dit* h, int32_t enable);

int gtav_dit_set_fused_temporal(gtav_dit* h, int32_t enable);

int gtav_dit_set_fused_spatial(gtav_dit* h, int32_t enable);
int gtav_dit_fused_launches(gtav_dit* h, int32_t B, int32_t T, int32_t t0);

int gtav_dit_set_weight_prefetch(gtav_dit* h, int32_t mode);

#define GTAV_PROFILE_CLASSES 9
int gtav_dit_profile(gtav_dit* h, int32_t enable);
int gtav_dit_profile_read(gtav_dit* h, double* ms_by_class, int64_t* launches_by_class);

int gtav_timer_calibrate(int32_t spin_us, int32_t reps, double* event_us_mean, double* device_us_mean, void* stream);

int gtav_dit_train_allow_window(gtav_dit* h, int32_t max_frames);
int gtav_dit_train_set_recompute(gtav_dit* h, int32_t enable);
int gtav_dit_train_saved_bytes(gtav_dit* h, int64_t* bytes);
int gtav_dit_train_param_count(gtav_dit* h, int64_t* numel);
int gtav_dit_train_enable(gtav_dit* h, float* grad_arena_dev, int64_t grad_arena_numel);
int gtav_dit_train_enable_typed(gtav_dit* h, float* grad_arena_dev, int64_t grad_arena_numel, int32_t dtype);
int gtav_dit_set_loss_scale(gtav_dit* h, float scale);
int gtav_dit_set_grad_divisor(gtav_dit* h, float divisor);
int gtav_dit_zero_grad(gtav_dit* h, void* stream);
int gtav_dit_train_forward(gtav_dit* h, const float* x_dev, const int64_t* t_dev, const float* actions_dev, float* out_dev,
                           int32_t B, int32_t T, void* stream);
int gtav_dit_train_backward(gtav_dit* h, const float* v_pred_dev, const float* v_target_dev, void* stream);
int gtav_dit_train_get_residual(gtav_dit* h, int32_t k, float* dst_dev, int64_t numel, void* stream);
int gtav_dit_train_backward_phases(gtav_dit* h, const float* v_pred_dev, const float* v_target_dev, int32_t phase_begin, int32_t phase_end,
                                   void* stream);
int gtav_dit_train_param_range(gtav_dit* h, const char* prefix, int64_t* offset, int64_t* count);
int gtav_dit_get_grad(gtav_dit* h, const char* name, float* dst_dev, int64_t numel, void* stream);
int gtav_dit_adamw_step(gtav_dit* h, float lr, float beta1, float beta2, float eps, float weight_decay, float max_grad_norm, void* stream);
int gtav_dit_train_stats(gtav_dit* h, float* out4_host, void* stream);
int gtav_dit_get_opt_state(gtav_dit* h, const char* name, float* m_dst_dev, float* v_dst_dev, int64_t numel, void* stream);
int gtav_dit_set_opt_state(gtav_dit* h, const char* name, const float* m_src_dev, const float* v_src_dev, int64_t numel, void* stream);
int gtav_dit_get_opt_step(gtav_dit* h, int64_t* applied_steps, int64_t* skipped_steps, void* stream);
int gtav_dit_set_opt_step(gtav_dit* h, int64_t applied_steps, int64_t skipped_steps, void* stream);

int gtav_dit_check(gtav_dit* h, void* stream);

#define GTAV_OPERAND_F16 0
#define GTAV_OPERAND_BF16 1
int gtav_dit_operand_groups(gtav_dit* h, int32_t* n_groups);
int gtav_dit_set_operand_dtype(gtav_dit* h, int32_t group, int32_t dtype);
int gtav_dit_get_operand_dtype(gtav_dit* h, int32_t group, int32_t* dtype);
int gtav_dit_autorange(gtav_dit* h, int32_t* n_switched, void* stream);

typedef struct gtav_vae_config {
    int32_t latent_dim, input_height, input_width, patch_size;
    int32_t enc_dim, enc_depth, enc_heads, dec_dim, dec_depth, dec_heads;
    float mlp_ratio;
    int32_t use_variational;
    int32_t max_frames_per_call;
} gtav_vae_config;

typedef struct gtav_vae gtav_vae;

int gtav_vae_create(const gtav_vae_config* cfg, gtav_vae** out);
void gtav_vae_destroy(gtav_vae* h);
int gtav_vae_set_weight(gtav_vae* h, const char* name, const float* src_dev, int64_t numel, void* stream);
// ... 97 lines not shown
```

### include/gtav_amd_testing.h

```cpp
#ifndef GTAV_AMD_TESTING_H
#define GTAV_AMD_TESTING_H

#include <stdint.h>

#ifdef __cplusplus
extern "C" {
#endif

void gtav_op_gemm_set_stages(int32_t ns);
void gtav_op_gemm_set_wm(int32_t wm);
void gtav_op_set_operand_dtype(int32_t dtype);
int gtav_op_attn_spatial_prescaled(const void* q, const void* k, const void* vt, void* o, int32_t NB, int32_t heads, int32_t S, void* stream);

#ifdef __cplusplus
}
#endif
#endif
```

Baseline: 5.316.

## Add per-class non-temporal weight fill policy and pass GEMM head params as scalar args

```diff
diff --git a/ai-generated-gtav_amd/csrc/api_dit.hip b/ai-generated-gtav_amd/csrc/api_dit.hip
--- a/ai-generated-gtav_amd/csrc/api_dit.hip
+++ b/ai-generated-gtav_amd/csrc/api_dit.hip
@@ -122,7 +122,10 @@
         const int pf_max_m = 1536;
         static const int pf_min_m = GTAV_ENV_INT("GTAV_PF_MIN_M", 256);
         on = h->w_prefetch && M >= pf_min_m && M <= pf_max_m;
-    }
+        fill_on = M <= pf_max_m;
+    }
+    bool fill_on;
+    int fill(int cls) const { return fill_on ? h->w_fill_cls[cls] : 0; }
     PrefetchDesc after(int hb, int pos) const {
         const int q = pos + 1, hb2 = hb + q / 4, consumer = (q + 3) % 4;
         if (!on || hb2 >= 2 * h->L) return kNoPrefetch;
@@ -174,7 +177,7 @@
         if (fused_t) rd.permute_rows(Tq, P);
         if (!folded_in) RET_IF(ln(ops, mb, mb + D, ef));
         GemmParams g = gemm_params(h->xn, D, fused_t || fused_s ? w.w_qkv_hm : w.w_qkv, M, 3 * D, D);
-        g.D = D; g.S = P; g.err_flag = ef; g.pf = pf.after(hb, 0);
+        g.D = D; g.S = P; g.err_flag = ef; g.pf = pf.after(hb, 0); g.wfill = pf.fill(3);
         if (folded_in) fold_consumer(h, g, 2 * hb, 3 * D, mod_rows, ctab);
         if (hf == 0) { g.qkv_mode = QKV_SPATIAL; g.rope_cs = h->rope_s.cs_dev; }
         else { g.qkv_mode = QKV_TEMPORAL; g.k = h->kvcache[l]; g.v = h->kvcache[l]; g.Tq = Tq; g.t0 = t0; g.Tmax = h->maxT; g.rope_cs = h->rope_t.cs_dev; }
@@ -191,13 +194,13 @@
         }
         folded_in = false;
         GemmParams fc1 = gemm_params(h->xn, D, w.w_fc1, M, h->Hm, D);
-        fc1.bias = w.b_fc1; fc1.out = h->hbuf; fc1.ldo = h->Hm_pad; fc1.err_flag = ef; fc1.pf = pf.after(hb, 2);
+        fc1.bias = w.b_fc1; fc1.out = h->hbuf; fc1.ldo = h->Hm_pad; fc1.err_flag = ef; fc1.pf = pf.after(hb, 2); fc1.wfill = pf.fill(1);
         if (fold_a) {
             RET_IF(fold_producer(h, PC_OUT, h->ao, w.w_out, M, D, w.b_out, gate(mb + 2 * D), mb + 4 * D, s));
             fold_consumer(h, fc1, 2 * hb + 1, h->Hm, mod_rows, ctab);
             PROF(h, PC_FC1, s, launch_gemm(fc1, EPI_GELU_TANH_FOLD, s));
         } else {
-            RET_IF(rd.gemm(ops, PC_OUT, h->ao, D, w.w_out, D, w.b_out, gate(mb + 2 * D), dit_resid_inplace(h, M, D), pf.after(hb, 1)));
+            RET_IF(rd.gemm(ops, PC_OUT, h->ao, D, w.w_out, D, w.b_out, gate(mb + 2 * D), dit_resid_inplace(h, M, D), pf.after(hb, 1), nullptr, nullptr, pf.fill(0)));
             RET_IF(ln(ops, mb + 3 * D, mb + 4 * D, ef));
             PROF(h, PC_FC1, s, ops.gemm(fc1, EPI_GELU_TANH, s));
         }
@@ -206,7 +209,7 @@
             RET_IF(fold_producer(h, PC_FC2, h->hbuf, w.w_fc2, M, h->Hm_pad, w.b_fc2, gate(mb + 5 * D), next_scale, s));
             folded_in = true;
         } else {
-            RET_IF(rd.gemm(ops, PC_FC2, h->hbuf, h->Hm_pad, w.w_fc2, h->Hm_pad, w.b_fc2, gate(mb + 5 * D), dit_resid_inplace(h, M, h->Hm_pad), pf.after(hb, 3)));
+            RET_IF(rd.gemm(ops, PC_FC2, h->hbuf, h->Hm_pad, w.w_fc2, h->Hm_pad, w.b_fc2, gate(mb + 5 * D), dit_resid_inplace(h, M, h->Hm_pad), pf.after(hb, 3), nullptr, nullptr, pf.fill(2)));
         }
     }
     const float* mf = mod + (size_t)h->L * 12 * D;
@@ -550,6 +553,18 @@
     return 0;
 }
 
+int gtav_dit_set_weight_fill_policy(gtav_dit* h, int32_t mode) {
+    GTAV_REQUIRE(h, "dit_set_weight_fill_policy: null handle");
+    GTAV_REQUIRE((mode & ~0x1111) == 0,
+                 "dit_set_weight_fill_policy: mode %d (one nibble per class: bits 0-3 out-proj's weight, 4-7 fc1's, 8-11 fc2's, 12-15 to_qkv's; "
+                 "nibble 0 = default cache policy, 1 = non-temporal fills)", mode);
+    int cls[4];
+    for (int c = 0; c < 4; ++c) cls[c] = (mode >> (4 * c)) & 15;
+    if (memcmp(cls, h->w_fill_cls, sizeof(cls))) h->drop_graphs();
+    memcpy(h->w_fill_cls, cls, sizeof(cls));
+    return 0;
+}
+
 #ifdef GTAV_EXPERIMENTS
 int gtav_dit_set_fold(gtav_dit* h, int32_t mode, int32_t min_tokens_a, int32_t min_tokens_b) {
     GTAV_REQUIRE(h && mode >= 0 && mode <= 2, "dit_set_fold: mode %d", mode);
diff --git a/ai-generated-gtav_amd/csrc/api_internal.h b/ai-generated-gtav_amd/csrc/api_internal.h
--- a/ai-generated-gtav_amd/csrc/api_internal.h
+++ b/ai-generated-gtav_amd/csrc/api_internal.h
@@ -257,9 +257,9 @@
     LnPending pend;
     bool pending = false;
     int gemm(const OperandOps& ops, int cls, const f16* X, int ldx, const f16* W, int K, const float* bias, const ResidGate& gt, bool inplace,
-             const PrefetchDesc& pf = kNoPrefetch, float* x_out = nullptr, f16* y_save = nullptr) {
+             const PrefetchDesc& pf = kNoPrefetch, float* x_out = nullptr, f16* y_save = nullptr, int wfill = 0) {
         GemmParams q = gemm_params(X, ldx, W, M, N, K);
-        q.out = parts; q.ldo = N; q.pf = pf;
+        q.out = parts; q.ldo = N; q.pf = pf; q.wfill = wfill;
         if (inplace) {
             q.out = resid; q.bias = bias; q.gate = gt.gate; q.gate_stride = gt.stride; q.gate_rows = gt.rows; q.rows_per_gate = gt.rows_per_gate;
         } else {
@@ -348,6 +348,7 @@
     bool fuse_sattn = false;
     bool w_prefetch = true;
     int w_prefetch_cls[4] = {1, 4, 4, 1};
+    int w_fill_cls[4] = {0, 0, 0, 0};
     int resid_inplace_min_m = GTAV_ENV_INT("GTAV_RESID_INPLACE_MIN_M", 1 << 30);
     struct Fold {
         bool geom_ok = false;
diff --git a/ai-generated-gtav_amd/csrc/elementwise.hip b/ai-generated-gtav_amd/csrc/elementwise.hip
--- a/ai-generated-gtav_amd/csrc/elementwise.hip
+++ b/ai-generated-gtav_amd/csrc/elementwise.hip
@@ -72,11 +72,13 @@
 #define LN_DBG(pd, b) false
 #endif
 template <int MODE, bool PEND, int KS = 0>
-__global__ __launch_bounds__(512) void ln_row_block_kernel(float* __restrict__ x, int ldx, f16* __restrict__ out, int M, int D,
+__global__ __launch_bounds__(512) void ln_row_block_kernel(float* __restrict__ x, int ldx, int D, const float* __restrict__ h_parts, size_t h_slab_stride, int h_ld,
+                                                           int h_nsplit, int h_flags, int rows_per_mod, f16* __restrict__ out, int M,
                                                            const float* __restrict__ p0, const float* __restrict__ p1,
-                                                           int mod_stride, const int* __restrict__ rows, int rows_per_mod,
+                                                           int mod_stride, const int* __restrict__ rows,
                                                            LnPending pd) {
     __shared__ float red[16];
+    pd.parts = h_parts; pd.slab_stride = h_slab_stride; pd.ld = h_ld; pd.nsplit = h_nsplit; pd.flags = h_flags;
     const int m = blockIdx.x;
     const int c = threadIdx.x * 4;
     const int nw = (blockDim.x + 63) >> 6, wid = threadIdx.x >> 6, lane = threadIdx.x & 63;
@@ -703,6 +705,7 @@
 
 #define LN_WAVE_ROW_(MODE, NV, P0, P1, STRIDE, ROWS, RPM) \
     GTAV_LAUNCH((ln_wave_row_kernel<MODE, NV>), dim3(cdiv(M, 4)), dim3(256), 0, stream, x, ldx, out, M, D, P0, P1, STRIDE, ROWS, RPM, pd_.flags, err_flag)
+#define LN_ROW_BLOCK_ARGS_(P0, P1, STRIDE, ROWS, RPM) x, ldx, D, pd_.parts, pd_.slab_stride, pd_.ld, pd_.nsplit, pd_.flags, RPM, out, M, P0, P1, STRIDE, ROWS, pd_
 #define LN_DISPATCH(MODE, P0, P1, STRIDE, ROWS, RPM)                                                     \
     do {                                                                                                  \
         LnPending pd_;                                                                                    \
@@ -716,8 +719,8 @@
         GTAV_REQUIRE(!pd_.k_load || !upd_, "ln: k_load excludes a pending update");                                                            \
         if (pd_.k_save || pd_.k_load) {                  \
             const dim3 g_(M), b_(round_up(D / 4, 64));                                                    \
-            if (pd_.k_save) GTAV_LAUNCH((ln_row_block_kernel<MODE, true, 1>), g_, b_, 0, stream, x, ldx, out, M, D, P0, P1, STRIDE, ROWS, RPM, pd_); \
-            else GTAV_LAUNCH((ln_row_block_kernel<MODE, false, 2>), g_, b_, 0, stream, x, ldx, out, M, D, P0, P1, STRIDE, ROWS, RPM, pd_);      \
+            if (pd_.k_save) GTAV_LAUNCH((ln_row_block_kernel<MODE, true, 1>), g_, b_, 0, stream, LN_ROW_BLOCK_ARGS_(P0, P1, STRIDE, ROWS, RPM)); \
+            else GTAV_LAUNCH((ln_row_block_kernel<MODE, false, 2>), g_, b_, 0, stream, LN_ROW_BLOCK_ARGS_(P0, P1, STRIDE, ROWS, RPM));      \
         } else if (!upd_ && pd_.tperm_T == 0 && M >= g_ln_wave_row_min && (D == 256 || D == 512 || D == 1024 || D == 2048)) { \
             if (D == 256) LN_WAVE_ROW_(MODE, 1, P0, P1, STRIDE, ROWS, RPM);                               \
             else if (D == 512) LN_WAVE_ROW_(MODE, 2, P0, P1, STRIDE, ROWS, RPM);                          \
@@ -725,8 +728,8 @@
             else LN_WAVE_ROW_(MODE, 8, P0, P1, STRIDE, ROWS, RPM);                                        \
         } else {                                                                   \
             const dim3 g_(M), b_(round_up(D / 4, 64));                                                    \
-            if (upd_) GTAV_LAUNCH((ln_row_block_kernel<MODE, true>), g_, b_, 0, stream, x, ldx, out, M, D, P0, P1, STRIDE, ROWS, RPM, pd_); \
-            else GTAV_LAUNCH((ln_row_block_kernel<MODE, false>), g_, b_, 0, stream, x, ldx, out, M, D, P0, P1, STRIDE, ROWS, RPM, pd_);     \
+            if (upd_) GTAV_LAUNCH((ln_row_block_kernel<MODE, true>), g_, b_, 0, stream, LN_ROW_BLOCK_ARGS_(P0, P1, STRIDE, ROWS, RPM)); \
+            else GTAV_LAUNCH((ln_row_block_kernel<MODE, false>), g_, b_, 0, stream, LN_ROW_BLOCK_ARGS_(P0, P1, STRIDE, ROWS, RPM));     \
         }                                                                                                 \
     } while (0)
 
diff --git a/ai-generated-gtav_amd/csrc/gemm.hip b/ai-generated-gtav_amd/csrc/gemm.hip
--- a/ai-generated-gtav_amd/csrc/gemm.hip
+++ b/ai-generated-gtav_amd/csrc/gemm.hip
@@ -23,6 +23,11 @@
 __device__ __forceinline__ void glds16_s(const void* sbase, unsigned voff, unsigned lds_addr) {
     unsigned keep;
     asm volatile("s_mov_b32 %0, m0\n\ts_mov_b32 m0, %3\n\ts_nop 0\n\tglobal_load_lds_dwordx4 %1, %2\n\ts_mov_b32 m0, %0"
+                 : "=&s"(keep) : "v"(voff), "s"(sbase), "s"(lds_addr) : "memory");
+}
+__device__ __forceinline__ void glds16_s_nt(const void* sbase, unsigned voff, unsigned lds_addr) {
+    unsigned keep;
+    asm volatile("s_mov_b32 %0, m0\n\ts_mov_b32 m0, %3\n\ts_nop 0\n\tglobal_load_lds_dwordx4 %1, %2 nt\n\ts_mov_b32 m0, %0"
                  : "=&s"(keep) : "v"(voff), "s"(sbase), "s"(lds_addr) : "memory");
 }
 __device__ __forceinline__ void store16_soff(const void* sbase, unsigned voff, u32x4 v) {
@@ -541,9 +546,9 @@
 
 __device__ __forceinline__ int div_rcp(int a, unsigned rcp) { return rcp ? (int)__umulhi((unsigned)a, rcp) : a; }
 template <bool SPLITK, int TNB, int TMB>
-__device__ __forceinline__ void tile_map_fast(const GemmParams& p, int& n0, int& m0, int& ks, int& kt0, int& nkt) {
+__device__ __forceinline__ void tile_map_fast(const GemmParams& p, int& n0, int& m0, int& ks, int& kt0, int& nkt, int nwg = (int)gridDim.x) {
     const GemmParams::TileMap& tm = p.tm;
-    const int nwg = gridDim.x, bid = blockIdx.x;
+    const int bid = blockIdx.x;
     const int xcd = bid & 7, qq = nwg >> 3, rr = nwg & 7;
     const int swz = (xcd < rr ? xcd * (qq + 1) : rr * (qq + 1) + (xcd - rr) * qq) + (bid >> 3);
     int tile_id = swz;
@@ -562,6 +567,18 @@
     n0 = tile_n * TNB;
     m0 = tile_m * TMB;
 }
+
+#define GTAV_HEAD_PARAMS unsigned h_rcp_group, int h_group, unsigned h_gn_tn, unsigned h_rcp_gn, unsigned h_rcp_gnlast, unsigned h_rcp_tiles, \
+                         const f16* h_W, const f16* h_X, int h_K, int h_N, int h_M, unsigned h_tiles_sk
+#define GTAV_HEAD_VALUES(q) (q).tm.rcp_group, (q).tm.group, (unsigned)(q).tm.gn | (unsigned)(q).tm.tiles_n << 16, (q).tm.rcp_gn, (q).tm.rcp_gnlast, (q).tm.rcp_tiles, \
+                            (q).W, (q).X, (q).K, (q).N, (q).M, (unsigned)(q).tm.tiles | (unsigned)(q).splitk << 16 | (unsigned)((q).wfill != 0) << 24
+#define GTAV_HEAD_APPLY(p)                                                                                                            \
+    do {                                                                                                                              \
+        (p).tm.rcp_group = h_rcp_group; (p).tm.group = h_group; (p).tm.gn = (int)(h_gn_tn & 0xFFFFu); (p).tm.tiles_n = (int)(h_gn_tn >> 16); \
+        (p).tm.rcp_gn = h_rcp_gn; (p).tm.rcp_gnlast = h_rcp_gnlast; (p).tm.rcp_tiles = h_rcp_tiles;                                   \
+        (p).W = h_W; (p).X = h_X; (p).K = h_K; (p).N = h_N; (p).M = h_M;                                                              \
+        (p).tm.tiles = (int)(h_tiles_sk & 0xFFFFu); (p).splitk = (int)(h_tiles_sk >> 16 & 0xFFu); (p).wfill = (int)(h_tiles_sk >> 24 & 1u); \
+    } while (0)
 
 constexpr int FOLD_NFR = 4;
 constexpr int fold_lds_bytes(int tnb) { return FOLD_NFR * 2 * tnb * 4; }
@@ -1604,11 +1621,13 @@
         const unsigned smem0 = lds_offset(smem);
         const char* sb[G];
         unsigned ldso[G];
+        unsigned wmask = 0;
 #pragma unroll
         for (int i = 0; i < G; ++i) {
             int q = lw * G + i;
             q = q < NP ? q : NP - 1;
             const bool isw = q < WPC;
+            wmask |= (unsigned)isw << i;
             const int row = isw ? n0 + 8 * q : m0 + 8 * (q - WPC);
             int rt = row >> 7;
             const int lim = isw ? last_wt : last_rt;
@@ -1624,6 +1643,26 @@
         };
         const int npro = nkt < NS - 1 ? nkt : NS - 1;
         GTAV_STAMP_SLOT(lw == 0 && lane == 0, 7);
+        if (p.wfill) {
+            auto stage_nt = [&](int t) {
+                const unsigned so = (unsigned)(t % NS) * STAGE_BYTES;
+                const size_t go = (size_t)t * TILE_BYTES;
+#pragma unroll
+                for (int i = 0; i < G; ++i) {
+                    if (wmask >> i & 1) glds16_s_nt(sb[i] + go, voff, ldso[i] + so);
+                    else glds16_s(sb[i] + go, voff, ldso[i] + so);
+                }
+            };
+            for (int t = 0; t < npro; ++t) stage_nt(t);
+            for (int t = 0; t < nkt; ++t) {
+                wait_vm_ring<NS, G>(nkt - 1 - t);
+                GTAV_STAMP_SLOT_HI(t == 0 && lw == 0 && lane == 0, 6);
+                wg_barrier();
+                if (t == 0) GTAV_STAMP(bs.t[1]);
+                if (t + NS - 1 < nkt) stage_nt(t + NS - 1);
+            }
+            return;
+        }
         for (int t = 0; t < npro; ++t) stage(t);
         for (int t = 0; t < nkt; ++t) {
             wait_vm_ring<NS, G>(nkt - 1 - t);
@@ -1736,7 +1775,7 @@
 }
 
 template <int EPIX, int NS, int FI, int FJ, int WN, int WM, int NL>
-__global__ __launch_bounds__(64 * (WN * WM + NL), 1) void gemm_l_kernel(GemmParams p) {
+__global__ __launch_bounds__(64 * (WN * WM + NL), 1) void gemm_l_kernel(GTAV_HEAD_PARAMS, GemmParams p) {
     constexpr int EPI = epi_base(EPIX);
     constexpr int TNB = 16 * FI * WN, TM = 16 * FJ * WM;
     constexpr int STAGE = (2 * FI * WN + 2 * FJ * WM) * 1024;
@@ -1745,16 +1784,12 @@
     extern __shared__ __attribute__((aligned(16))) char smem_l[];
     static_assert(NS * STAGE >= EPIB, "the ring must cover the epilogue's LDS image");
     char* smem = smem_l;
-#define GTAV_PIN_S(x) asm volatile("" ::"s"(x))
-    GTAV_PIN_S(p.X); GTAV_PIN_S(p.W); GTAV_PIN_S(p.M); GTAV_PIN_S(p.N); GTAV_PIN_S(p.K); GTAV_PIN_S(p.splitk);
-    GTAV_PIN_S(p.tm.tiles_m); GTAV_PIN_S(p.tm.tiles_n); GTAV_PIN_S(p.tm.gn); GTAV_PIN_S(p.tm.group); GTAV_PIN_S(p.tm.tiles);
-    GTAV_PIN_S(p.tm.rcp_tiles); GTAV_PIN_S(p.tm.rcp_group); GTAV_PIN_S(p.tm.rcp_gn); GTAV_PIN_S(p.tm.rcp_gnlast);
-    GTAV_PIN_S(p.bias); GTAV_PIN_S(p.out); GTAV_PIN_S(p.ldo); GTAV_PIN_S(p.qkv_mode); GTAV_PIN_S(p.D);
-#undef GTAV_PIN_S
+    GTAV_HEAD_APPLY(p);
+    auto pin_args = [&]() { asm volatile("" ::"s"(p.bias), "s"(p.out), "s"(p.ldo), "s"(p.qkv_mode), "s"(p.D)); };
     BlockStamps bs;
     bs.begin(p);
     int n0, m0, ks, kt0, nkt;
-    tile_map_fast<EPI == EPI_PARTIAL, TNB, TM>(p, n0, m0, ks, kt0, nkt);
+    tile_map_fast<EPI == EPI_PARTIAL, TNB, TM>(p, n0, m0, ks, kt0, nkt, EPI == EPI_PARTIAL ? p.tm.tiles * p.splitk : p.tm.tiles);
     f32x4 acc[FI][FJ];
 #pragma unroll
     for (int i = 0; i < FI; ++i)
@@ -1774,6 +1809,7 @@
         tr = (p.qkv_mode == QKV_SPATIAL) && (n0 >= 2 * p.D);
         f32x4 prope[FI][FJ];
         auto pfq = [&]() {
+            pin_args();
             prefetch_bias<EPI, FI, WM, WN, NL>(p, n0, pbias);
             prefetch_rope<FI, FJ, WM, WN, NL>(p, n0, m0, prope);
             pff();
@@ -1784,19 +1820,19 @@
         epilogue<EPIX, FI, FJ, WM, WN, NL, true>(p, acc, pbias, smem, n0, m0, ks, tr, prope, ft);
     } else if constexpr (EPI == EPI_QKV) {
         tr = (p.qkv_mode == QKV_SPATIAL) && (n0 >= 2 * p.D);
-        auto pf = [&]() { prefetch_bias<EPI, FI, WM, WN, NL>(p, n0, pbias); pff(); };
+        auto pf = [&]() { pin_args(); prefetch_bias<EPI, FI, WM, WN, NL>(p, n0, pbias); pff(); };
         if (tr) mainloop_l<true, NS, FI, FJ, WN, WM, NL>(p, smem, n0, m0, kt0, nkt, acc, bs, pf);
         else mainloop_l<false, NS, FI, FJ, WN, WM, NL>(p, smem, n0, m0, kt0, nkt, acc, bs, pf);
         GTAV_STAMP(bs.t[2]);
         epilogue<EPIX, FI, FJ, WM, WN, NL, false>(p, acc, pbias, smem, n0, m0, ks, tr, acc, ft);
     } else if constexpr (FOLDP) {
         f32x4 xpre[FI][FJ];
-        auto pf = [&]() { prefetch_bias<EPI, FI, WM, WN, NL>(p, n0, pbias); prefetch_resid<FI, FJ, WM, WN, NL>(p, n0, m0, xpre, 0, FI * FJ); };
+        auto pf = [&]() { pin_args(); prefetch_bias<EPI, FI, WM, WN, NL>(p, n0, pbias); prefetch_resid<FI, FJ, WM, WN, NL>(p, n0, m0, xpre, 0, FI * FJ); };
         mainloop_l<false, NS, FI, FJ, WN, WM, NL>(p, smem, n0, m0, kt0, nkt, acc, bs, pf);
         GTAV_STAMP(bs.t[2]);
         epilogue<EPIX, FI, FJ, WM, WN, NL, true>(p, acc, pbias, smem, n0, m0, ks, tr, xpre, ft);
     } else {
-        auto pf = [&]() { prefetch_bias<EPI, FI, WM, WN, NL>(p, n0, pbias); pff(); };
+        auto pf = [&]() { pin_args(); prefetch_bias<EPI, FI, WM, WN, NL>(p, n0, pbias); pff(); };
         mainloop_l<false, NS, FI, FJ, WN, WM, NL>(p, smem, n0, m0, kt0, nkt, acc, bs, pf);
         GTAV_STAMP(bs.t[2]);
         epilogue<EPIX, FI, FJ, WM, WN, NL, false>(p, acc, pbias, smem, n0, m0, ks, tr, acc, ft);
@@ -1805,21 +1841,17 @@
 }
 
 template <int NS>
-__global__ __launch_bounds__(512, 1) void gemm_qkvt_attn_kernel(GemmParams p) {
+__global__ __launch_bounds__(512, 1) void gemm_qkvt_attn_kernel(GTAV_HEAD_PARAMS, GemmParams p) {
     constexpr int FI = 3, FJ = 5, WN = 4, WM = 1, NL = 4, TNB = 192, TM = 80, TMAX = 5;
     constexpr int PN = 384;
     extern __shared__ __attribute__((aligned(16))) char smem_l[];
     static_assert(NS * (2 * FI * WN + 2 * FJ * WM) * 1024 >= TM * PN, "the ring must cover the epilogue's LDS image");
     char* smem = smem_l;
-#define GTAV_PIN_S(x) asm volatile("" ::"s"(x))
-    GTAV_PIN_S(p.X); GTAV_PIN_S(p.W); GTAV_PIN_S(p.M); GTAV_PIN_S(p.N); GTAV_PIN_S(p.K);
-    GTAV_PIN_S(p.tm.tiles_m); GTAV_PIN_S(p.tm.tiles_n); GTAV_PIN_S(p.tm.gn); GTAV_PIN_S(p.tm.group); GTAV_PIN_S(p.tm.tiles);
-    GTAV_PIN_S(p.tm.rcp_group); GTAV_PIN_S(p.tm.rcp_gn); GTAV_PIN_S(p.tm.rcp_gnlast);
-#undef GTAV_PIN_S
+    GTAV_HEAD_APPLY(p);
     BlockStamps bs;
     bs.begin(p);
     int n0, m0, ks, kt0, nkt;
-    tile_map_fast<false, TNB, TM>(p, n0, m0, ks, kt0, nkt);
+    tile_map_fast<false, TNB, TM>(p, n0, m0, ks, kt0, nkt, p.tm.tiles);
     f32x4 acc[FI][FJ];
 #pragma unroll
     for (int i = 0; i < FI; ++i)
@@ -1919,7 +1951,7 @@
 
 
 template <int NS>
-__global__ __launch_bounds__(768, 1) void gemm_qkvs_attn_kernel(GemmParams p) {
+__global__ __launch_bounds__(768, 1) void gemm_qkvs_attn_kernel(GTAV_HEAD_PARAMS, GemmParams p) {
     constexpr int FI = 3, FJ = 5, WN = 4, WM = 2, NL = 4, TNB = 192, TM = 144, NQT = TM / 16, NK = 10;
     constexpr int S_pad = 16 * NK, vstride = (S_pad + 8) * 2;
     constexpr int QS = 0, KS = TM * 128, VS = KS + S_pad * 128, IMG = VS + 64 * vstride;
@@ -1927,15 +1959,11 @@
     static_assert(NS * (2 * FI * WN + 2 * FJ * WM) * 1024 >= IMG, "the ring must cover the epilogue's LDS image");
     static_assert(16 * FJ * WM >= TM && 16 * FJ * WM == S_pad, "two token halves cover the frame");
     char* smem = smem_l;
-#define GTAV_PIN_S(x) asm volatile("" ::"s"(x))
-    GTAV_PIN_S(p.X); GTAV_PIN_S(p.W); GTAV_PIN_S(p.M); GTAV_PIN_S(p.N); GTAV_PIN_S(p.K);
-    GTAV_PIN_S(p.tm.tiles_m); GTAV_PIN_S(p.tm.tiles_n); GTAV_PIN_S(p.tm.gn); GTAV_PIN_S(p.tm.group); GTAV_PIN_S(p.tm.tiles);
-    GTAV_PIN_S(p.tm.rcp_group); GTAV_PIN_S(p.tm.rcp_gn); GTAV_PIN_S(p.tm.rcp_gnlast);
-#undef GTAV_PIN_S
+    GTAV_HEAD_APPLY(p);
     BlockStamps bs;
     bs.begin(p);
     int n0, m0, ks, kt0, nkt;
-    tile_map_fast<false, TNB, TM>(p, n0, m0, ks, kt0, nkt);
+    tile_map_fast<false, TNB, TM>(p, n0, m0, ks, kt0, nkt, p.tm.tiles);
     const int tid = threadIdx.x, lane = tid & 63, wraw = tid >> 6, w = wraw - NL, li = lane & 15, g = lane >> 4;
     const int wn = w & (WN - 1), wm = w >> 2;
     f32x4 acc[FI][FJ];
@@ -2214,7 +2242,8 @@
 static thread_local int g_force_stages = 0, g_force_wm = GTAV_ENV_INT("GTAV_GEMM_SHAPE", 0);
 static int g_debug = GTAV_ENV_INT("GTAV_GEMM_DEBUG", 0);
 void gemm_set_stages(int ns) { g_force_stages = ns; }
-void gemm_set_wm(int wm) { g_force_wm = wm; }
+static thread_local int g_force_wfill = 0;
+void gemm_set_wm(int wm) { g_force_wm = wm & 0xFF; g_force_wfill = wm >> 8 & 1; }
 #ifdef GTAV_EXPERIMENTS
 void gemm_set_debug(int bits) { g_debug = bits; }
 static unsigned long long* g_stamps = nullptr;
@@ -2320,8 +2349,9 @@
     }
     GemmParams q = p;
     if (int rc_ = fill_tile_map(q.tm, p.M, p.N, p.K, 16 * FJ * WM, 16 * FI * WN, splitk)) return rc_;
+    GTAV_REQUIRE(q.splitk >= 0 && q.splitk < 256, "gemm: %d K slices do not fit the launch-head arguments", q.splitk);
     const dim3 grid(q.tm.tiles * splitk);
-    GTAV_LAUNCH((gemm_l_kernel<EPI, NS, FI, FJ, WN, WM, NL>), grid, dim3(64 * (WN * WM + NL)), LDS, stream, q);
+    GTAV_LAUNCH((gemm_l_kernel<EPI, NS, FI, FJ, WN, WM, NL>), grid, dim3(64 * (WN * WM + NL)), LDS, stream, GTAV_HEAD_VALUES(q), q);
     GTAV_CHECK_HIP(hipGetLastError());
     return 0;
 }
@@ -2451,8 +2481,9 @@
 #endif
     q.out_sc1 = 1;
     q.splitk = 1;
+    if (g_force_wfill) q.wfill = 1;
     if (int rc_ = fill_tile_map(q.tm, q.M, q.N, q.K, 80, 192, 1)) return rc_;
-    GTAV_LAUNCH((gemm_qkvt_attn_kernel<NS>), dim3(q.tm.tiles), dim3(512), LDS, stream, q);
+    GTAV_LAUNCH((gemm_qkvt_attn_kernel<NS>), dim3(q.tm.tiles), dim3(512), LDS, stream, GTAV_HEAD_VALUES(q), q);
     GTAV_CHECK_HIP(hipGetLastError());
     return 0;
 }
@@ -2479,9 +2510,10 @@
     q.stamps = g_stamps;
 #endif
     q.splitk = 1;
+    if (g_force_wfill) q.wfill = 1;
     q.qkv_mode = QKV_SPATIAL;
     if (int rc_ = fill_tile_map(q.tm, q.M, q.N, q.K, 144, 192, 1)) return rc_;
-    GTAV_LAUNCH((gemm_qkvs_attn_kernel<NS>), dim3(q.tm.tiles), dim3(768), LDS, stream, q);
+    GTAV_LAUNCH((gemm_qkvs_attn_kernel<NS>), dim3(q.tm.tiles), dim3(768), LDS, stream, GTAV_HEAD_VALUES(q), q);
     GTAV_CHECK_HIP(hipGetLastError());
     return 0;
 }
@@ -2582,6 +2614,7 @@
     p.stamps = g_stamps;
 #endif
     p.out_sc1 = (g_debug & 8) ? 0 : 1;
+    if (g_force_wfill) p.wfill = 1;
     GTAV_REQUIRE(prefetch_desc_ok(p.pf), "gemm: bad prefetch descriptor (row tiles %d, K tiles %d, K slices %d)", p.pf.rt, p.pf.nkt, p.pf.splitk);
     if (g_debug & 0x800000) p.pf.next = nullptr;
     GTAV_REQUIRE(p.K > 0 && p.K % TK == 0, "gemm: K=%d must be a positive multiple of %d", p.K, TK);
diff --git a/ai-generated-gtav_amd/csrc/gemm_typed.inc b/ai-generated-gtav_amd/csrc/gemm_typed.inc
--- a/ai-generated-gtav_amd/csrc/gemm_typed.inc
+++ b/ai-generated-gtav_amd/csrc/gemm_typed.inc
@@ -1,6 +1,7 @@
 struct GemmParams {
     const f16* X;
     int ldx;
+    int wfill;
     const f16* W;
     int M, N, K;
     int debug;
diff --git a/ai-generated-gtav_amd/generate.py b/ai-generated-gtav_amd/generate.py
--- a/ai-generated-gtav_amd/generate.py
+++ b/ai-generated-gtav_amd/generate.py
@@ -100,9 +100,15 @@
     return 0x10000 | cls[0] | cls[1] << 4 | cls[2] << 8 | cls[3] << 12
 
 
+def fill_policy_mode(cls) -> int:
+    if any(v not in (0, 1) for v in cls) or len(cls) != 4:
+        raise ValueError(f"fill_policy_mode: {cls!r} is not four values of 0 / 1")
+    return cls[0] | cls[1] << 4 | cls[2] << 8 | cls[3] << 12
+
+
 @torch.inference_mode()
 def tune_weight_prefetch(model, B: int = 1, window: Optional[int] = None, steps: int = 24, rounds: int = 2, use_actions: bool = False,
-                         latent_hw=None, per_class: bool = True, fused_temporal: bool = True, fused_spatial: bool = True) -> dict:
+                         latent_hw=None, per_class: bool = True, fused_temporal: bool = True, fused_spatial: bool = True, fill_policy: bool = True) -> dict:
     dev = model.device
     T = int(window or model.max_frames)
     h, w = latent_hw or (model.input_h, model.input_w)
@@ -175,9 +181,26 @@
         timed(cur)
         fused_s = {"on_ms": round(t_on, 4), "off_ms": round(t_off, 4), "chosen": "on" if keep else "off", "was": was}
         cur_ms = min(cur_ms, t_on) if keep else cur_ms
+    fill = None
+    if fill_policy and B * T * (h // model.patch_size) * (w // model.patch_size) <= 1536:
+        fcur, fms = [0, 0, 0, 0], {}
+        for c in (2, 1, 0, 3):
+            t_keep = t_nt = float("inf")
+            cand = fcur[:c] + [1] + fcur[c + 1:]
+            for _ in range(rounds):
+                model.set_weight_fill_policy(fill_policy_mode(fcur))
+                t_keep = min(t_keep, timed(cur))
+                model.set_weight_fill_policy(fill_policy_mode(cand))
+                t_nt = min(t_nt, timed(cur))
+            fms[PREFETCH_CLASSES[c]] = [round(t_keep, 4), round(t_nt, 4)]
+            if t_nt < t_keep * 0.997:
+                fcur, cur_ms = cand, min(cur_ms, t_nt)
+        model.set_weight_fill_policy(fill_policy_mode(fcur))
+        timed(cur)
+        fill = {"classes": dict(zip(PREFETCH_CLASSES, fcur)), "mode": fill_policy_mode(fcur), "ms": fms}
     model.check()
     chosen = "on" if cur == on else "off" if cur == off else "per-class"
-    return {"on_ms": round(best[on], 4), "off_ms": round(best[off], 4), "chosen": chosen, "classes": dict(zip(PREFETCH_CLASSES, cur)),
+    return {"weight_fill_policy": fill, "on_ms": round(best[on], 4), "off_ms": round(best[off], 4), "chosen": chosen, "classes": dict(zip(PREFETCH_CLASSES, cur)),
             "mode": prefetch_mode(cur), "tuned_ms": round(cur_ms, 4), "fused_temporal_qkv_attention": fused, "fused_spatial_qkv_attention": fused_s}
 
 
diff --git a/ai-generated-gtav_amd/lib.py b/ai-generated-gtav_amd/lib.py
--- a/ai-generated-gtav_amd/lib.py
+++ b/ai-generated-gtav_amd/lib.py
@@ -88,6 +88,7 @@
     "gtav_dit_set_fused_spatial": [_p, _i],
     "gtav_dit_fused_launches": [_p, _i, _i, _i],
     "gtav_dit_set_weight_prefetch": [_p, _i],
+    "gtav_dit_set_weight_fill_policy": [_p, _i],
     "gtav_dit_profile": [_p, _i],
     "gtav_dit_profile_read": [_p, C.POINTER(C.c_double), C.POINTER(C.c_int64)],
     "gtav_timer_calibrate": [_i, _i, C.POINTER(C.c_double), C.POINTER(C.c_double), _p],
diff --git a/ai-generated-gtav_amd/model/dit.py b/ai-generated-gtav_amd/model/dit.py
--- a/ai-generated-gtav_amd/model/dit.py
+++ b/ai-generated-gtav_amd/model/dit.py
@@ -262,6 +262,8 @@
                     _lib.check(L.gtav_dit_set_fold(self._handle, *self._fold))
                 if getattr(self, "_weight_prefetch", None) is not None:
                     _lib.check(L.gtav_dit_set_weight_prefetch(self._handle, int(self._weight_prefetch)))
+                if getattr(self, "_weight_fill_policy", None) is not None:
+                    _lib.check(L.gtav_dit_set_weight_fill_policy(self._handle, int(self._weight_fill_policy)))
                 for g in sorted(self._bf16_groups):
                     _lib.check(L.gtav_dit_set_operand_dtype(self._handle, g, 1))
                 if self._trainable:
@@ -516,6 +518,14 @@
         if self._handle:
             _lib.check(_lib.load().gtav_dit_set_weight_prefetch(self._handle, mode))
 
+    def set_weight_fill_policy(self, mode: int):
+        mode = int(mode)
+        if mode & ~0x1111:
+            raise ValueError(f"set_weight_fill_policy: mode {mode:#x} is not a per-class word of nibbles 0 / 1 (gtav_amd.generate.fill_policy_mode)")
+        self._weight_fill_policy = mode
+        if self._handle:
+            _lib.check(_lib.load().gtav_dit_set_weight_fill_policy(self._handle, mode))
+
     def set_fold(self, mode: int, min_tokens_a: int = -1, min_tokens_b: int = -1):
         if not getattr(_lib.load(), "_gtav_experiments", False):
             raise _lib.GtavError("set_fold: the LayerNorm fold exists only in the experiments build (gtav_amd.lib.load_experiments())")
diff --git a/include/gtav_amd.h b/include/gtav_amd.h
--- a/include/gtav_amd.h
+++ b/include/gtav_amd.h
@@ -45,6 +45,8 @@
 int gtav_dit_fused_launches(gtav_dit* h, int32_t B, int32_t T, int32_t t0);
 
 int gtav_dit_set_weight_prefetch(gtav_dit* h, int32_t mode);
+
+int gtav_dit_set_weight_fill_policy(gtav_dit* h, int32_t mode);
 
 #define GTAV_PROFILE_CLASSES 9
 int gtav_dit_profile(gtav_dit* h, int32_t enable);
diff --git a/include/gtav_amd_testing.h b/include/gtav_amd_testing.h
--- a/include/gtav_amd_testing.h
+++ b/include/gtav_amd_testing.h
@@ -2,6 +2,8 @@
 #define GTAV_AMD_TESTING_H
 
 #include <stdint.h>
+
+#define GTAV_GEMM_WM_NT_WEIGHT_FILLS 0x100
 
 #ifdef __cplusplus
 extern "C" {
```

Measured after the change: 5.646 (median of 6 runs). 6.2% higher.
